# mokemokechicken/reversi-alpha-zero

Measured on NVIDIA H100. Metric: self_play_games_per_sec, higher is better.
Workload: dtype f16

## Files before the change

include/rz_engine.h:

```cpp
#ifndef RZ_ENGINE_H
#define RZ_ENGINE_H

#include <stddef.h>
#include <stdint.h>

#ifdef __cplusplus
extern "C" {
#endif

#define RZ_OK 0
#define RZ_EINVAL (-1)
#define RZ_ECUDA (-2)
#define RZ_ENOMEM (-3)
#define RZ_ESTATE (-4)
#define RZ_ECAPACITY (-5)
#define RZ_EIO (-6)

#define RZ_ABI_VERSION 2

int rz_abi_version(void);
const char* rz_last_error(void);
int rz_device_count(int* count);


int rz_find_correct_moves_dev(const uint64_t* own, const uint64_t* enemy, uint64_t* out, size_t n, void* stream);
int rz_find_correct_moves(const uint64_t* own, const uint64_t* enemy, uint64_t* out, size_t n);

int rz_calc_flip_dev(const uint8_t* pos, const uint64_t* own, const uint64_t* enemy, uint64_t* out, size_t n, void* stream);
int rz_calc_flip(const uint8_t* pos, const uint64_t* own, const uint64_t* enemy, uint64_t* out, size_t n);

int rz_step_dev(uint64_t* black, uint64_t* white, uint8_t* next_player, uint8_t* turn, uint8_t* done,
                uint8_t* winner, const int8_t* action, uint64_t* legal_out, size_t n, void* stream);
int rz_step(uint64_t* black, uint64_t* white, uint8_t* next_player, uint8_t* turn, uint8_t* done,
            uint8_t* winner, const int8_t* action, uint64_t* legal_out, size_t n);

int rz_dihedral_dev(const uint64_t* x, const uint8_t* t, uint64_t* out, size_t n, void* stream);

int rz_solve_dev(const uint64_t* own, const uint64_t* enemy, const uint8_t* exactly, int8_t* move, int8_t* score, size_t n,
                 void* stream);
int rz_solve(const uint64_t* own, const uint64_t* enemy, const uint8_t* exactly, int8_t* move, int8_t* score, size_t n);

typedef struct rz_deep_solve_stats {
    int32_t probes;
    int32_t slices;
    int32_t resplits;
    int32_t pad;
    int64_t leaves;
    int64_t node_steps;
    double seconds;
} rz_deep_solve_stats;
int rz_solve_deep(const uint64_t* own, const uint64_t* enemy, int8_t* move, int8_t* score, size_t n, double timeout_s,
                  rz_deep_solve_stats* stats);
int rz_solve_deep_tune(int slice_us, int leaf_target, int leaf_floor);

typedef struct rz_env_state {
    uint64_t black, white;
    uint8_t next_player, turn, done, winner;
} rz_env_state;
uint64_t rz_find_correct_moves_host(uint64_t own, uint64_t enemy);
uint64_t rz_calc_flip_host(int pos, uint64_t own, uint64_t enemy);
uint64_t rz_dihedral_host(uint64_t x, int t);
int rz_bitsliced_host(const uint8_t* pos, const uint64_t* own, const uint64_t* enemy, uint64_t* out, size_t n);
void rz_env_reset_host(rz_env_state* s);
void rz_env_update_host(rz_env_state* s, uint64_t black, uint64_t white, int next_player);
void rz_env_step_host(rz_env_state* s, int action );

typedef struct rz_net rz_net;

typedef struct rz_net_cfg {
    int32_t filters;
    int32_t res_blocks;
    int32_t value_fc;
    int32_t kernel_size;
} rz_net_cfg;

#define RZ_NET_IMPL_AUTO 0
#define RZ_NET_IMPL_GENERIC 1
#define RZ_NET_IMPL_TCGEN05 2
#define RZ_NET_IMPL_SPLIT 3

int rz_net_set_tower_cluster(int cluster);
int rz_net_create(const rz_net_cfg* cfg, int device, rz_net** out);
int rz_net_destroy(rz_net* net);
int rz_net_blob_size(const rz_net* net, size_t* n_floats);
int rz_net_load_weights(rz_net* net, const float* blob_host, size_t n_floats);
int rz_net_load_weights_dev(rz_net* net, const float* blob_dev, size_t n_floats, void* stream);

int rz_net_predict_dev(rz_net* net, const uint64_t* own, const uint64_t* enemy, float* policy, float* value,
                       size_t n, int impl, void* stream);
int rz_net_predict_counted_dev(rz_net* net, const uint64_t* own, const uint64_t* enemy, float* policy, float* value,
                               const uint32_t* count_dev, size_t max_n, int impl, void* stream);
int rz_net_debug_tower_dev(rz_net* net, const uint64_t* own, const uint64_t* enemy, float* policy, float* value,
                           float* tower, size_t n, void* stream);
int rz_net_debug_heads_dev(rz_net* net, const uint64_t* own, const uint64_t* enemy, float* policy, float* value,
                           float* tower, float* policy_logits, float* value_logit, size_t n, void* stream);
int rz_net_debug_heads_impl_dev(rz_net* net, const uint64_t* own, const uint64_t* enemy, float* policy, float* value,
                                float* tower, float* policy_logits, float* value_logit, size_t n, int impl, void* stream);
int rz_net_select_impl(const rz_net* net, size_t n, int* impl);
int rz_net_predict(rz_net* net, const uint8_t* planes, float* policy, float* value, size_t n, int impl);

typedef struct rz_engine rz_engine;

#define RZ_EVAL_NET 0
#define RZ_EVAL_FAKE 1

typedef struct rz_engine_cfg {
    int32_t games;
    int32_t simulation_num_per_move;
    int32_t parallel_search_num;
    int32_t virtual_loss;
    int32_t change_tau_turn;
    int32_t thinking_loop;
    int32_t required_visit_to_decide_action;
    int32_t start_rethinking_turn;
    int32_t allowed_resign_turn;
    int32_t use_resign_threshold;
    int32_t share_mtcs_info;
    int32_t eval_mode;
    int32_t net_impl;
    int32_t max_plies;
    int32_t warm_start;
    int32_t overlap_groups;
    int32_t max_sims_per_wave;
    int32_t use_solver_turn;
    int32_t use_solver_turn_in_simulation;
    int32_t reset_mtcs_info_per_game;
    int32_t max_searches_per_game;
    int32_t arena_simulation_num;
    int32_t eval_cache_mb;
    float c_puct;
    float noise_eps;
    float dirichlet_alpha;
    float resign_threshold;
    float disable_resignation_rate;
    uint64_t seed;
    uint64_t first_game_id;
    uint64_t game_id_stride;
    uint64_t max_games;
} rz_engine_cfg;

typedef struct rz_ply {
    uint64_t own, enemy;
    int32_t n_visit[64];
    int16_t action;
    uint8_t player;
    uint8_t loops;
    uint8_t recorded;
    uint8_t pad;
    uint16_t waves;
    float n;
    float q;
} rz_ply;

typedef struct rz_game {
    uint64_t game_id;
    uint64_t black, white;
    int32_t first_ply;
    int32_t n_plies;
    int32_t expansions;
    int32_t simulations;
    uint8_t winner;
    int8_t black_z;
    uint8_t resign_enabled;
    uint8_t resigned_mask;
    uint8_t turn;
    uint8_t black_net;
    uint8_t pad[2];
    int32_t table_nodes;
    int32_t pad2;
} rz_game;

typedef struct rz_stats {
    uint64_t games_started, games_finished;
    uint64_t expansions;
    uint64_t simulations;
    uint64_t waves;
    uint64_t plies;
    uint64_t nn_launches, mcts_launches;
    uint64_t max_nodes_used, max_edges_used;
    double nn_ms, mcts_ms;
    double run_ms;
    uint64_t tower_rows;
    uint64_t cache_lookups;
    uint64_t cache_hits;
    uint64_t cache_repeats;
} rz_stats;

int rz_engine_create(const rz_engine_cfg* cfg, rz_net* net , int device,
                     rz_engine** out);
int rz_engine_destroy(rz_engine* e);
int rz_engine_run(rz_engine* e, uint64_t finished_target, uint64_t max_waves);
int rz_engine_poll(rz_engine* e, rz_game* games, size_t game_cap, size_t* n_games, rz_ply* plies, size_t ply_cap,
                   size_t* n_plies);
int rz_engine_stats(rz_engine* e, rz_stats* out);
int rz_engine_cache_turn_stats(rz_engine* e, uint64_t* lookups, uint64_t* hits, int n);
int rz_engine_set_max_games(rz_engine* e, uint64_t max_games);
int rz_engine_set_warm_start_profile(rz_engine* e, const float* weight, int n);
int rz_engine_set_simulation_num(rz_engine* e, int32_t sims);
int rz_engine_set_second_net(rz_engine* e, rz_net* net_b, int enable);
int rz_engine_set_resign_threshold(rz_engine* e, int use_resign_threshold, float resign_threshold);
int rz_engine_search_root(rz_engine* e, uint64_t own, uint64_t enemy, int player, int slot, int keep_tree,
                          int32_t* n_visit, float* w_sum);

int rz_write_play_data(const char* path, const rz_game* games, size_t n_games, const rz_ply* plies,
                       int save_policy_of_tau_1, int change_tau_turn, size_t* n_records);

typedef struct rz_play_row {
    uint64_t own, enemy;
    int32_t n_visit[64];
    int32_t z;
    int32_t pad;
} rz_play_row;

int rz_write_play_rows(const char* path, const rz_game* games, size_t n_games, const rz_ply* plies,
                       int save_policy_of_tau_1, int change_tau_turn, size_t* n_rows);
int rz_read_play_rows(const char* path, rz_play_row* rows, size_t capacity, size_t* n_rows,
                      int* save_policy_of_tau_1, int* change_tau_turn);
int rz_ingest_dev(const rz_play_row* rows, size_t n_rows, int save_policy_of_tau_1, int change_tau_turn,
                  uint8_t* planes, float* policy, float* z, void* stream);
int rz_ingest(const rz_play_row* rows, size_t n_rows, int save_policy_of_tau_1, int change_tau_turn,
              uint8_t* planes, float* policy, float* z);

int rz_ingest_json_dev(const char* text, size_t n_bytes, size_t capacity, uint8_t* planes, float* policy, float* z,
                       size_t* n_records, size_t* error_offset, void* stream);
int rz_ingest_json_host(const char* text, size_t n_bytes, size_t capacity, uint8_t* planes, float* policy, float* z,
                        size_t* n_records, size_t* error_offset);
int rz_ingest_json(const char* path, size_t capacity, uint8_t* planes, float* policy, float* z, size_t* n_records,
                   size_t* error_offset);

typedef struct rz_trainer rz_trainer;

typedef struct rz_train_cfg {
    int32_t max_batch;
    float momentum;
    float l2_reg;
    float bn_momentum;
} rz_train_cfg;

int rz_trainer_create(const rz_net_cfg* net, const rz_train_cfg* cfg, int device, rz_trainer** out);
int rz_trainer_create_group(const rz_net_cfg* net, const rz_train_cfg* cfg, const int* devices, int n_devices, rz_trainer** out);
int rz_train_shard_plan_host(int filters, int res_blocks, int batch, int n_devices, int32_t* bounds);
int rz_trainer_destroy(rz_trainer* t);
int rz_trainer_blob_size(const rz_trainer* t, size_t* n_floats);
int rz_trainer_load_weights(rz_trainer* t, const float* blob_host, size_t n_floats);
int rz_trainer_load_weights_dev(rz_trainer* t, const float* blob_dev, size_t n_floats, void* stream);
int rz_trainer_weights_dev(rz_trainer* t, float* blob_dev, size_t n_floats, void* stream);
int rz_trainer_step_dev(rz_trainer* t, const uint8_t* planes, const float* policy, const float* z, size_t n_records,
                        const int32_t* index, size_t batch, float lr, float* loss_dev, void* stream);
int rz_trainer_last_grad_dev(rz_trainer* t, float* grad_dev, size_t n_floats, void* stream);
int rz_trainer_replica_state_dev(rz_trainer* t, int r, float* blob_dev, float* vel_dev, size_t n_floats, void* stream);

#define RZ_TRAIN_CONV0_FWD 0
#define RZ_TRAIN_CONV_FWD 1
#define RZ_TRAIN_CONV_DGRAD 2
#define RZ_TRAIN_CONV_WGRAD 3
#define RZ_TRAIN_CONV0_WGRAD 4
int rz_trainer_debug_conv_dev(rz_trainer* t, int op, const float* in, const float* kernel, const float* bias, const float* add,
                              size_t batch, float* out, void* stream);

#define RZ_TRAIN_T_X0 0
#define RZ_TRAIN_T_Y 1
#define RZ_TRAIN_T_A 2
#define RZ_TRAIN_T_STATS 3
#define RZ_TRAIN_T_STAT 4
#define RZ_TRAIN_T_HC 5
#define RZ_TRAIN_T_AH 6
#define RZ_TRAIN_T_DH 7
#define RZ_TRAIN_T_DYH 8
#define RZ_TRAIN_T_HP 9
#define RZ_TRAIN_T_HV 10
#define RZ_TRAIN_T_DL 11
#define RZ_TRAIN_T_H1 12
#define RZ_TRAIN_T_DH1 13
#define RZ_TRAIN_T_DV 14
#define RZ_TRAIN_T_LP 15
#define RZ_TRAIN_T_LV 16
#define RZ_TRAIN_T_LOSS_PV 17
#define RZ_TRAIN_T_G 18
#define RZ_TRAIN_T_DY 19
#define RZ_TRAIN_T_DZ 20
int rz_trainer_debug_tensor_dev(rz_trainer* t, int which, int layer, float* out, size_t n_floats, void* stream);
int rz_trainer_debug_keep_backward(rz_trainer* t, int on);

#ifdef __cplusplus
}
#endif
#endif
```

reversi-alpha-zero_b200/csrc/rz_net.cu:

```cuda
#include <math.h>
#include <stdlib.h>
#include <string.h>
#include <new>
#include "rz_bitboard.cuh"
#include "rz_net.cuh"
#include "rz_tc_common.cuh"

namespace rz {

constexpr float kBnEps = 1e-3f;

__global__ void fold_bn_kernel(const float* __restrict__ blob, size_t group_off, size_t kernel_floats, int cout,
                               float* __restrict__ scale, float* __restrict__ shift) {
    int c = blockIdx.x * blockDim.x + threadIdx.x;
    if (c >= cout) return;
    const float* p = blob + group_off + kernel_floats;
    float bias = p[c], gamma = p[cout + c], beta = p[2 * cout + c], mean = p[3 * cout + c], var = p[4 * cout + c];
    float s = gamma / sqrtf(var + kBnEps);
    scale[c] = s;
    shift[c] = beta + (bias - mean) * s;
}

constexpr int kGThreads = 256;

template <int PIX>
__device__ __forceinline__ void conv3x3_layer(const float* __restrict__ in, float* __restrict__ out, const float* __restrict__ w,
                                              const float* __restrict__ scale, const float* __restrict__ shift, int cin, int F,
                                              bool add_residual, int oc, int pg, bool active) {
    float acc[PIX];
#pragma unroll
    for (int i = 0; i < PIX; ++i) acc[i] = 0.f;
    if (active) {
        for (int ci = 0; ci < cin; ++ci) {
            const float* inc = in + ci * 100;
#pragma unroll
            for (int tap = 0; tap < 9; ++tap) {
                const float wv = __ldg(w + ((size_t)tap * cin + ci) * F + oc);
                const int dy = tap / 3, dx = tap % 3;
#pragma unroll
                for (int i = 0; i < PIX; ++i) {
                    const int p = pg * PIX + i;
                    acc[i] = fmaf(inc[((p >> 3) + dy) * 10 + (p & 7) + dx], wv, acc[i]);
                }
            }
        }
        const float s = scale[oc], b = shift[oc];
#pragma unroll
        for (int i = 0; i < PIX; ++i) {
            const int p = pg * PIX + i;
            const int o = oc * 100 + ((p >> 3) + 1) * 10 + (p & 7) + 1;
            float y = fmaf(acc[i], s, b);
            if (add_residual) y += out[o];
            out[o] = fmaxf(y, 0.f);
        }
    }
}

template <int PIX>
__global__ void __launch_bounds__(kGThreads) net_generic_kernel(const float* __restrict__ blob, const float* __restrict__ ss,
                                                                rz_net net, const u64* __restrict__ own, const u64* __restrict__ enemy,
                                                                float* __restrict__ policy, float* __restrict__ value, size_t n,
                                                                const uint32_t* __restrict__ n_dev) {
    extern __shared__ float smem[];
    if (n_dev) n = *n_dev;
    const int F = net.cfg.filters, R = net.cfg.res_blocks, V = net.cfg.value_fc;
    float* bufA = smem;
    float* bufB = smem + F * 100;
    float* hp = bufB + F * 100;
    float* hv = hp + 128;
    float* fc = hv + 64;
    const int t = threadIdx.x;
    constexpr int NPG = 64 / PIX;
    const int oc = t % F, pg = t / F;
    const bool active = (t < F * NPG) && (pg < NPG);

    for (size_t pos = blockIdx.x; pos < n; pos += gridDim.x) {
        for (int i = t; i < 2 * F * 100; i += kGThreads) smem[i] = 0.f;
        __syncthreads();
        const u64 o = own[pos], e = enemy[pos];
        if (t < 128) {
            const int c = t >> 6, p = t & 63;
            bufB[c * 100 + ((p >> 3) + 1) * 10 + (p & 7) + 1] = (float)(((c ? e : o) >> p) & 1ULL);
        }
        __syncthreads();
        conv3x3_layer<PIX>(bufB, bufA, blob + net.off_conv0, ss, ss + F, 2, F, false, oc, pg, active);
        __syncthreads();
        for (int r = 0; r < R; ++r) {
            const float* w1 = blob + net.off_res0 + (size_t)(2 * r) * net.res_stride_conv;
            const float* w2 = w1 + net.res_stride_conv;
            const float* ss1 = ss + (size_t)(1 + 2 * r) * 2 * F;
            const float* ss2 = ss1 + 2 * F;
            conv3x3_layer<PIX>(bufA, bufB, w1, ss1, ss1 + F, F, F, false, oc, pg, active);
            __syncthreads();
            conv3x3_layer<PIX>(bufB, bufA, w2, ss2, ss2 + F, F, F, true, oc, pg, active);
            __syncthreads();
        }
        const float* ssh = ss + (size_t)(1 + 2 * R) * 2 * F;
        if (t < 192) {
            const int c = t >> 6, p = t & 63;
            const float* w = c < 2 ? blob + net.off_policy_conv + c : blob + net.off_value_conv;
            const int wstride = c < 2 ? 2 : 1;
            float acc = 0.f;
            const int o2 = ((p >> 3) + 1) * 10 + (p & 7) + 1;
            for (int ci = 0; ci < F; ++ci) acc = fmaf(bufA[ci * 100 + o2], __ldg(w + (size_t)ci * wstride), acc);
            if (c < 2) hp[c * 64 + p] = fmaxf(fmaf(acc, ssh[c], ssh[2 + c]), 0.f);
            else       hv[p] = fmaxf(fmaf(acc, ssh[4], ssh[5]), 0.f);
        }
        __syncthreads();
        if (t < 64) {
            const float* k = blob + net.off_policy_fc_k;
            float acc = __ldg(blob + net.off_policy_fc_b + t);
            for (int i = 0; i < 128; ++i) acc = fmaf(hp[i], __ldg(k + i * 64 + t), acc);
            fc[t] = acc;
        }
        __syncthreads();
        if (t < 64) {
            float m = -INFINITY;
            for (int i = 0; i < 64; ++i) m = fmaxf(m, fc[i]);
            float sum = 0.f;
            for (int i = 0; i < 64; ++i) sum += expf(fc[i] - m);
            policy[pos * 64 + t] = expf(fc[t] - m) / sum;
        }
        __syncthreads();
        for (int j = t; j < V; j += kGThreads) {
            const float* k = blob + net.off_value_fc1_k;
            float acc = __ldg(blob + net.off_value_fc1_b + j);
            for (int i = 0; i < 64; ++i) acc = fmaf(hv[i], __ldg(k + (size_t)i * V + j), acc);
            fc[j] = fmaxf(acc, 0.f);
        }
        __syncthreads();
        if (t == 0) {
            float acc = __ldg(blob + net.off_value_fc2_b);
            for (int j = 0; j < V; ++j) acc = fmaf(fc[j], __ldg(blob + net.off_value_fc2_k + j), acc);
            value[pos] = tanhf(acc);
        }
        __syncthreads();
    }
}

int net_forward_generic(rz_net* net, const uint64_t* own, const uint64_t* enemy, float* policy, float* value, size_t n,
                        cudaStream_t stream, const uint32_t* n_dev) {
    const int F = net->cfg.filters, V = net->cfg.value_fc;
    RZ_REQUIRE(F >= 2 && F <= 256, "generic kernel supports 2 <= filters <= 256 (got %d)", F);
    const size_t smem = ((size_t)2 * F * 100 + 128 + 64 + (V > 64 ? V : 64)) * sizeof(float);
    int npg = kGThreads / F;
    int pix = 64;
    while (pix > 4 && 64 / (pix / 2) <= npg) pix /= 2;
    size_t blocks = n < (size_t)num_sms() * 2 ? n : (size_t)num_sms() * 2;
    if (smem > 110 * 1024) blocks = n < (size_t)num_sms() ? n : (size_t)num_sms();
#define RZ_LAUNCH_G(P)                                                                                             \
    do {                                                                                                           \
        RZ_CUDA_TRY(cudaFuncSetAttribute(net_generic_kernel<P>, cudaFuncAttributeMaxDynamicSharedMemorySize, (int)smem)); \
        net_generic_kernel<P><<<(unsigned)blocks, kGThreads, smem, stream>>>(net->blob, net->scale_shift, *net, own, enemy, policy, value, n, n_dev); \
    } while (0)
    switch (pix) {
        case 64: RZ_LAUNCH_G(64); break;
        case 32: RZ_LAUNCH_G(32); break;
        case 16: RZ_LAUNCH_G(16); break;
        case 8: RZ_LAUNCH_G(8); break;
        default: RZ_LAUNCH_G(4); break;
    }
#undef RZ_LAUNCH_G
    RZ_LAUNCH_CHECK();
    return RZ_OK;
}

constexpr size_t kSplitMaxBatch = 0;

int select_impl(const rz_net* net, size_t n, int impl) {
    if (impl != RZ_NET_IMPL_AUTO) return impl;
    if (!tc_width(net->cfg.filters) || net->cfg.value_fc > (int)tc::kTcMaxV) return RZ_NET_IMPL_GENERIC;
    if (net->cfg.filters != 256) return RZ_NET_IMPL_TCGEN05;
    return n <= kSplitMaxBatch ? RZ_NET_IMPL_SPLIT : RZ_NET_IMPL_TCGEN05;
}

int net_forward(rz_net* net, const uint64_t* own, const uint64_t* enemy, float* policy, float* value, size_t n, int impl,
                cudaStream_t stream) {
    if (!net->loaded) { set_error("rz_net: weights not loaded"); return RZ_ESTATE; }
    if (n == 0) return RZ_OK;
    impl = select_impl(net, n, impl);
    if (impl == RZ_NET_IMPL_TCGEN05 || impl == RZ_NET_IMPL_SPLIT) {
        if (impl == RZ_NET_IMPL_SPLIT) {
            RZ_REQUIRE(net->cfg.filters == 256, "the split tower requires filters == 256 (got %d)", net->cfg.filters);
            return net_forward_split(net, own, enemy, policy, value, n, stream, nullptr);
        }
        RZ_REQUIRE(tc_width(net->cfg.filters), "the tensor-core tower requires filters 64, 128 or 256 (got %d)", net->cfg.filters);
        return net_forward_tc(net, own, enemy, policy, value, n, stream, nullptr);
    }
    RZ_REQUIRE(impl == RZ_NET_IMPL_GENERIC, "unknown net impl %d", impl);
    return net_forward_generic(net, own, enemy, policy, value, n, stream);
}

int net_forward_counted(rz_net* net, const uint64_t* own, const uint64_t* enemy, float* policy, float* value,
                        const uint32_t* count_dev, size_t max_n, int impl, cudaStream_t stream) {
    if (!net->loaded) { set_error("rz_net: weights not loaded"); return RZ_ESTATE; }
    impl = select_impl(net, max_n, impl);
    if (impl == RZ_NET_IMPL_TCGEN05) return net_forward_tc(net, own, enemy, policy, value, max_n, stream, nullptr, count_dev);
    if (impl == RZ_NET_IMPL_SPLIT) return net_forward_split(net, own, enemy, policy, value, max_n, stream, nullptr, count_dev);
    return net_forward_generic(net, own, enemy, policy, value, max_n, stream, count_dev);
}

static int finish_load(rz_net* net, cudaStream_t stream) {
    const rz_net_cfg& c = net->cfg;
    const int F = c.filters, L = n_conv_layers(c);
    float* ss = net->scale_shift;
    for (int l = 0; l < L; ++l) {
        const size_t off = l == 0 ? net->off_conv0 : net->off_res0 + (size_t)(l - 1) * net->res_stride_conv;
        const size_t kf = l == 0 ? (size_t)9 * 2 * F : (size_t)9 * F * F;
        fold_bn_kernel<<<(F + 127) / 128, 128, 0, stream>>>(net->blob, off, kf, F, ss + (size_t)l * 2 * F, ss + (size_t)l * 2 * F + F);
    }
    float* ssh = ss + (size_t)L * 2 * F;
    fold_bn_kernel<<<1, 32, 0, stream>>>(net->blob, net->off_policy_conv, (size_t)F * 2, 2, ssh, ssh + 2);
    fold_bn_kernel<<<1, 32, 0, stream>>>(net->blob, net->off_value_conv, (size_t)F, 1, ssh + 4, ssh + 5);
    RZ_LAUNCH_CHECK();
    if (F == 256) RZ_TRY(net_pack_tc(net, stream));
    else if (tc_width(F)) RZ_TRY(net_pack_tc_narrow(net, stream));
    RZ_CUDA_TRY(cudaStreamSynchronize(stream));
    net->loaded = true;
    net->weights_version++;
    return RZ_OK;
}

}

using namespace rz;

extern "C" {

int rz_net_create(const rz_net_cfg* cfg, int device, rz_net** out) {
    RZ_REQUIRE(cfg && out, "rz_net_create: null pointer");
    RZ_REQUIRE(cfg->kernel_size == 3, "only cnn_filter_size == 3 is supported (got %d)", cfg->kernel_size);
    RZ_REQUIRE(cfg->filters >= 2 && cfg->filters <= 256 && cfg->res_blocks >= 0 && cfg->res_blocks <= 64 && cfg->value_fc >= 1 &&
                   cfg->value_fc <= 4096,
               "unsupported model configuration (filters=%d res_blocks=%d value_fc=%d)", cfg->filters, cfg->res_blocks, cfg->value_fc);
    RZ_CUDA_TRY(cudaSetDevice(device));
    rz_net* net = new (std::nothrow) rz_net();
    if (!net) { set_error("out of host memory"); return RZ_ENOMEM; }
    memset(net, 0, sizeof(*net));
    net->cfg = *cfg;
    net->device = device;
    const size_t F = cfg->filters, V = cfg->value_fc, R = cfg->res_blocks;
    size_t off = 0;
    net->off_conv0 = off; off += 9 * 2 * F + 5 * F;
    net->off_res0 = off; net->res_stride_conv = 9 * F * F + 5 * F; off += 2 * R * net->res_stride_conv;
    net->off_policy_conv = off; off += F * 2 + 5 * 2;
    net->off_policy_fc_k = off; off += 128 * 64;
    net->off_policy_fc_b = off; off += 64;
    net->off_value_conv = off; off += F + 5;
    net->off_value_fc1_k = off; off += 64 * V;
    net->off_value_fc1_b = off; off += V;
    net->off_value_fc2_k = off; off += V;
    net->off_value_fc2_b = off; off += 1;
    net->blob_floats = off;
    cudaError_t e = cudaMalloc(&net->blob, off * sizeof(float));
    if (e == cudaSuccess) e = cudaMalloc(&net->scale_shift, ss_floats(*cfg) * sizeof(float));
    if (e == cudaSuccess && tc_width((int)F)) {
        e = cudaMalloc(&net->tc_w0, (size_t)4 * F * 8 * sizeof(__half));
        if (e == cudaSuccess && R > 0) e = cudaMalloc(&net->tc_w, (size_t)2 * R * 9 * F * F * sizeof(__half));
        if (e == cudaSuccess) e = cudaMalloc(&net->res, (size_t)num_sms() * kTowerResFloatsPerCta * sizeof(float));
        if (e == cudaSuccess) e = cudaEventCreateWithFlags(&net->res_done, cudaEventDisableTiming);
    }
    if (e != cudaSuccess) {
        set_error("rz_net_create: cudaMalloc failed: %s", cudaGetErrorString(e));
        cudaGetLastError();
        rz_net_destroy(net);
        return RZ_ENOMEM;
    }
    *out = net;
    return RZ_OK;
}

int rz_net_destroy(rz_net* net) {
    if (!net) return RZ_OK;
    cudaSetDevice(net->device);
    cudaFree(net->blob); cudaFree(net->scale_shift); cudaFree(net->tc_w0); cudaFree(net->tc_w); cudaFree(net->scratch);
    cudaFree(net->res); cudaFree(net->feat);
    if (net->res_done) cudaEventDestroy(net->res_done);
    delete net;
    return RZ_OK;
}

int rz_net_blob_size(const rz_net* net, size_t* n_floats) {
    RZ_REQUIRE(net && n_floats, "rz_net_blob_size: null pointer");
    *n_floats = net->blob_floats;
    return RZ_OK;
}

int rz_net_load_weights(rz_net* net, const float* blob_host, size_t n_floats) {
    RZ_REQUIRE(net && blob_host, "rz_net_load_weights: null pointer");
    RZ_REQUIRE(n_floats == net->blob_floats, "weight blob has %zu floats, this configuration needs %zu", n_floats, net->blob_floats);
    RZ_CUDA_TRY(cudaSetDevice(net->device));
    RZ_CUDA_TRY(cudaMemcpy(net->blob, blob_host, n_floats * sizeof(float), cudaMemcpyHostToDevice));
    return finish_load(net, 0);
}

int rz_net_load_weights_dev(rz_net* net, const float* blob_dev, size_t n_floats, void* stream) {
    RZ_REQUIRE(net && blob_dev, "rz_net_load_weights_dev: null pointer");
    RZ_REQUIRE(n_floats == net->blob_floats, "weight blob has %zu floats, this configuration needs %zu", n_floats, net->blob_floats);
    RZ_CUDA_TRY(cudaSetDevice(net->device));
    RZ_CUDA_TRY(cudaMemcpyAsync(net->blob, blob_dev, n_floats * sizeof(float), cudaMemcpyDeviceToDevice, (cudaStream_t)stream));
    return finish_load(net, (cudaStream_t)stream);
}

int rz_net_set_tower_cluster(int cluster) { return set_tower_cluster(cluster); }

int rz_net_predict_dev(rz_net* net, const uint64_t* own, const uint64_t* enemy, float* policy, float* value, size_t n, int impl,
                       void* stream) {
    RZ_REQUIRE(net && (n == 0 || (own && enemy && policy && value)), "rz_net_predict_dev: null pointer");
    return net_forward(net, own, enemy, policy, value, n, impl, (cudaStream_t)stream);
}

int rz_net_predict_counted_dev(rz_net* net, const uint64_t* own, const uint64_t* enemy, float* policy, float* value,
                               const uint32_t* count_dev, size_t max_n, int impl, void* stream) {
    RZ_REQUIRE(net && count_dev && (max_n == 0 || (own && enemy && policy && value)), "rz_net_predict_counted_dev: null pointer");
    if (max_n == 0) return RZ_OK;
    return net_forward_counted(net, own, enemy, policy, value, count_dev, max_n, impl, (cudaStream_t)stream);
}

int rz_net_debug_tower_dev(rz_net* net, const uint64_t* own, const uint64_t* enemy, float* policy, float* value, float* tower, size_t n,
                           void* stream) {
    RZ_REQUIRE(net && own && enemy && policy && value && tower, "rz_net_debug_tower_dev: null pointer");
    if (!net->loaded) { set_error("rz_net: weights not loaded"); return RZ_ESTATE; }
    return net_forward_tc(net, own, enemy, policy, value, n, (cudaStream_t)stream, tower);
}

int rz_net_debug_heads_dev(rz_net* net, const uint64_t* own, const uint64_t* enemy, float* policy, float* value, float* tower,
                           float* policy_logits, float* value_logit, size_t n, void* stream) {
    RZ_REQUIRE(net && own && enemy && policy && value && policy_logits && value_logit, "rz_net_debug_heads_dev: null pointer");
    if (!net->loaded) { set_error("rz_net: weights not loaded"); return RZ_ESTATE; }
    return net_forward_tc(net, own, enemy, policy, value, n, (cudaStream_t)stream, tower, nullptr, policy_logits, value_logit);
}

int rz_net_debug_heads_impl_dev(rz_net* net, const uint64_t* own, const uint64_t* enemy, float* policy, float* value, float* tower,
                                float* policy_logits, float* value_logit, size_t n, int impl, void* stream) {
    RZ_REQUIRE(net && own && enemy && policy && value && policy_logits && value_logit, "rz_net_debug_heads_impl_dev: null pointer");
    if (!net->loaded) { set_error("rz_net: weights not loaded"); return RZ_ESTATE; }
    RZ_REQUIRE(tc_width(net->cfg.filters), "the tensor-core tower requires filters 64, 128 or 256 (got %d)", net->cfg.filters);
    if (n == 0) return RZ_OK;
    impl = select_impl(net, n, impl);
    if (impl == RZ_NET_IMPL_SPLIT)
        return net_forward_split(net, own, enemy, policy, value, n, (cudaStream_t)stream, tower, nullptr, policy_logits, value_logit);
    RZ_REQUIRE(impl == RZ_NET_IMPL_TCGEN05, "rz_net_debug_heads_impl_dev: impl must be AUTO, TCGEN05 or SPLIT (got %d)", impl);
    return net_forward_tc(net, own, enemy, policy, value, n, (cudaStream_t)stream, tower, nullptr, policy_logits, value_logit);
}

int rz_net_select_impl(const rz_net* net, size_t n, int* impl) {
    RZ_REQUIRE(net && impl, "rz_net_select_impl: null pointer");
    *impl = select_impl(net, n, RZ_NET_IMPL_AUTO);
    return RZ_OK;
}

int rz_net_predict(rz_net* net, const uint8_t* planes, float* policy, float* value, size_t n, int impl) {
    RZ_REQUIRE(net && (n == 0 || (planes && policy && value)), "rz_net_predict: null pointer");
    if (n == 0) return RZ_OK;
    RZ_CUDA_TRY(cudaSetDevice(net->device));
    const size_t need = n * (16 + 65 * 4) + 256;
    if (need > net->scratch_bytes) {
        cudaFree(net->scratch); net->scratch = nullptr; net->scratch_bytes = 0;
        RZ_CUDA_TRY(cudaMalloc(&net->scratch, need));
        net->scratch_bytes = need;
    }
    uint64_t* hb = (uint64_t*)malloc(n * 16);
    if (!hb) { set_error("out of host memory"); return RZ_ENOMEM; }
    for (size_t i = 0; i < n; ++i) {
        uint64_t o = 0, e = 0;
        const uint8_t* p = planes + i * 128;
        for (int b = 0; b < 64; ++b) { o |= (uint64_t)(p[b] != 0) << b; e |= (uint64_t)(p[64 + b] != 0) << b; }
        hb[i] = o; hb[n + i] = e;
    }
    uint64_t* d_own = (uint64_t*)net->scratch;
    uint64_t* d_en = d_own + n;
    float* d_pol = (float*)(d_en + n);
    float* d_val = d_pol + n * 64;
    cudaError_t ce = cudaMemcpyAsync(d_own, hb, n * 16, cudaMemcpyHostToDevice, 0);
    int rc = RZ_OK;
    if (ce == cudaSuccess) rc = net_forward(net, d_own, d_en, d_pol, d_val, n, impl, 0);
    if (ce == cudaSuccess && rc == RZ_OK) ce = cudaMemcpyAsync(policy, d_pol, n * 64 * sizeof(float), cudaMemcpyDeviceToHost, 0);
    if (ce == cudaSuccess && rc == RZ_OK) ce = cudaMemcpyAsync(value, d_val, n * sizeof(float), cudaMemcpyDeviceToHost, 0);
    if (ce == cudaSuccess && rc == RZ_OK) ce = cudaStreamSynchronize(0);
    free(hb);
    if (rc != RZ_OK) return rc;
    if (ce != cudaSuccess) { set_error("rz_net_predict: %s", cudaGetErrorString(ce)); return RZ_ECUDA; }
    return RZ_OK;
}

}
```

reversi-alpha-zero_b200/csrc/rz_net.cuh:

```cuda
#pragma once
#include <cuda_fp16.h>
#include <mutex>
#include "rz_common.cuh"

struct rz_net {
    rz_net_cfg cfg;
    int device;
    bool loaded;
    uint64_t weights_version;
    size_t blob_floats;
    float* blob;
    float* scale_shift;
    size_t off_conv0, off_res0, res_stride_conv;
    size_t off_policy_conv, off_policy_fc_k, off_policy_fc_b;
    size_t off_value_conv, off_value_fc1_k, off_value_fc1_b, off_value_fc2_k, off_value_fc2_b;
    __half* tc_w0;
    __half* tc_w;
    float* res;
    cudaEvent_t res_done;
    float* feat;
    size_t feat_rows;
    void* scratch;
    size_t scratch_bytes;
};

namespace rz {

constexpr size_t kTowerResFloatsPerCta = 256 * 128;
constexpr int kHeadFeatures = 192;

inline int n_conv_layers(const rz_net_cfg& c) { return 1 + 2 * c.res_blocks; }
inline size_t ss_floats(const rz_net_cfg& c) { return (size_t)n_conv_layers(c) * 2 * c.filters + 4 + 2; }

int net_forward_generic(rz_net* net, const uint64_t* own, const uint64_t* enemy, float* policy, float* value, size_t n,
                        cudaStream_t stream, const uint32_t* n_dev = nullptr);
int net_forward_counted(rz_net* net, const uint64_t* own, const uint64_t* enemy, float* policy, float* value,
                        const uint32_t* count_dev, size_t max_n, int impl, cudaStream_t stream);
int net_forward_tc(rz_net* net, const uint64_t* own, const uint64_t* enemy, float* policy, float* value, size_t n,
                   cudaStream_t stream, float* dbg_tower ,
                   const uint32_t* n_dev = nullptr ,
                   float* dbg_logits = nullptr , float* dbg_vlogit = nullptr );
int net_forward_split(rz_net* net, const uint64_t* own, const uint64_t* enemy, float* policy, float* value, size_t n,
                      cudaStream_t stream, float* dbg_tower, const uint32_t* n_dev = nullptr, float* dbg_logits = nullptr,
                      float* dbg_vlogit = nullptr);
int select_impl(const rz_net* net, size_t n, int impl);
int net_pack_tc(rz_net* net, cudaStream_t stream);
std::mutex& tower_mutex();
int head_features(rz_net* net, size_t n);
int net_forward_tc_narrow(rz_net* net, const uint64_t* own, const uint64_t* enemy, float* policy, float* value, size_t n,
                          cudaStream_t stream, float* dbg_tower, const uint32_t* n_dev, float* dbg_logits, float* dbg_vlogit);
int net_pack_tc_narrow(rz_net* net, cudaStream_t stream);
inline bool tc_width(int filters) { return filters == 64 || filters == 128 || filters == 256; }
int set_tower_cluster(int cluster);
int tower_cluster();
int net_forward(rz_net* net, const uint64_t* own, const uint64_t* enemy, float* policy, float* value, size_t n, int impl,
                cudaStream_t stream);

}
```

reversi-alpha-zero_b200/csrc/rz_net_tc.cu:

```cuda
#include <stdlib.h>
#include <mutex>
#include <type_traits>
#include "rz_bitboard.cuh"
#include "rz_net.cuh"
#include "rz_tc_common.cuh"

namespace rz {
namespace tc {

constexpr int kThreads = 384;
constexpr uint32_t kProducerRegs = 40, kMathRegs = 232;
constexpr int kMathThreads = 256;
constexpr uint32_t kActCg = 2896, kActSlot = 144;
constexpr uint32_t kActBytes = 32 * kActCg;
constexpr uint32_t kStageBytes = 32768, kStages = 3;
constexpr int kResAhead = 4;
constexpr uint32_t kA0Bytes = 8192, kW0Bytes = 16384;
constexpr uint32_t kOffAct = 0;
constexpr uint32_t kOffW = kOffAct + kActBytes;
constexpr uint32_t kOffA0 = kOffW + kStages * kStageBytes;
constexpr uint32_t kOffW0 = kOffA0 + kA0Bytes;
constexpr uint32_t kOffSS = kOffW0 + kW0Bytes;
constexpr uint32_t kOffHw = kOffSS + 2 * 2048;
constexpr uint32_t kOffBar = kOffHw + 768 * 4;
constexpr uint32_t kNumBars = 2 * kStages + 1;
constexpr uint32_t kSmemBytes = kOffBar + kNumBars * 8;
constexpr uint32_t kSmemAlloc = kSmemBytes + 128;
static_assert(kSmemAlloc <= 232448, "shared memory budget exceeded");
static_assert(kTowerResFloatsPerCta == (size_t)kMathThreads * 128, "residual scratch per CTA");

#ifdef RZ_TOWER_STAMPS
enum : int {
    kStTiles,
    kStTile,
    kStKLoop,
    kStFull,
    kStMma,
    kStEpiBar,
    kStEpi0,
    kStEpi1,
    kStEpi2,
    kStEpiLast,
    kStFeat,
    kStEmpty,
    kStCount
};
constexpr int kStMaxCtas = 1024;
__device__ unsigned long long g_tower_stamps[kStMaxCtas][kStCount];
__device__ __forceinline__ void stamp_add(int phase, uint32_t cycles) { atomicAdd(&g_tower_stamps[blockIdx.x][phase], (unsigned long long)cycles); }
#define RZ_STAMP(...) __VA_ARGS__
#else
#define RZ_STAMP(...)
#endif

template <int CL>
__global__ void __launch_bounds__(kThreads, 1) net_tower_kernel(const Params pp) {
    Params p = pp;
    if (p.n_dev) p.n = *p.n_dev;
    extern __shared__ uint8_t smem_raw[];
    const uint32_t base = (smem_u32(smem_raw) + 127u) & ~127u;
    uint8_t* sm = smem_raw + (base - smem_u32(smem_raw));
    const int warp = threadIdx.x >> 5, lane = threadIdx.x & 31;
    const uint32_t bar0 = base + kOffBar;
    auto bar_full = [&](uint32_t s) { return bar0 + s * 8; };
    auto bar_empty = [&](uint32_t s) { return bar0 + (kStages + s) * 8; };
    const uint32_t bar_w0 = bar0 + 2 * kStages * 8;
    const uint32_t ntiles = (p.n + 1) >> 1;
    const int L = p.n_layers;
    const uint32_t crank = CL > 1 ? cluster_ctarank() : 0u;
    const uint32_t cbase = blockIdx.x - crank;
    const uint32_t iters = cbase < ntiles ? (ntiles - cbase + gridDim.x - 1) / gridDim.x : 0u;

    for (uint32_t i = threadIdx.x * 16; i < kActBytes; i += kThreads * 16) *reinterpret_cast<uint4*>(sm + kOffAct + i) = make_uint4(0, 0, 0, 0);
    fence_proxy_async();
    for (uint32_t i = threadIdx.x; i < 768; i += kThreads)
        reinterpret_cast<float*>(sm + kOffHw)[i] = __ldg(i < 512 ? p.blob + p.off_policy_conv + i : p.blob + p.off_value_conv + (i - 512));
    if (threadIdx.x == 0) {
        for (uint32_t s = 0; s < kStages; ++s) { mbar_init(bar_full(s), 1); mbar_init(bar_empty(s), 8 * CL); }
        mbar_init(bar_w0, 1);
        asm volatile("fence.mbarrier_init.release.cluster;" ::: "memory");
    }
    __syncthreads();
    if (CL > 1) cluster_sync_all();

    if (warp >= 8) {
        asm volatile("setmaxnreg.dec.sync.aligned.u32 %0;" ::"n"(kProducerRegs));
        if (warp == 8 && lane == 0) {
            if (iters > 0) {
                mbar_expect_tx(bar_w0, kW0Bytes);
                bulk_g2s(base + kOffW0, p.w0, kW0Bytes, bar_w0);
            }
            uint32_t stage = 0, phase = 0;
            for (uint32_t it = 0; it < iters; ++it) {
                for (int l = 1; l < L; ++l) {
                    const uint8_t* src = reinterpret_cast<const uint8_t*>(p.w) + (size_t)(l - 1) * 36 * kStageBytes;
                    RZ_STAMP(uint32_t st_empty = 0;)
                    for (int s = 0; s < 36; ++s) {
                        RZ_STAMP(const uint32_t c0 = (uint32_t)clock();)
                        mbar_wait(bar_empty(stage), phase ^ 1);
                        RZ_STAMP(st_empty += (uint32_t)clock() - c0;)
                        mbar_expect_tx(bar_full(stage), kStageBytes);
                        if (CL == 1) {
                            bulk_g2s(base + kOffW + stage * kStageBytes, src + (size_t)s * kStageBytes, kStageBytes, bar_full(stage));
                        } else {
                            constexpr uint32_t kSlice = kStageBytes / CL;
                            bulk_g2s_mc(base + kOffW + stage * kStageBytes + crank * kSlice, src + (size_t)s * kStageBytes + crank * kSlice,
                                        kSlice, bar_full(stage), (uint16_t)((1u << CL) - 1u));
                        }
                        if (++stage == kStages) { stage = 0; phase ^= 1; }
                    }
                    RZ_STAMP(stamp_add(kStEmpty, st_empty);)
                }
            }
        }
    } else {
        asm volatile("setmaxnreg.inc.sync.aligned.u32 %0;" ::"n"(kMathRegs));
        const int et = threadIdx.x;
        const int wg = warp >> 2;
        const int r0 = wg * 64 + (warp & 3) * 16 + (lane >> 2);
        const int g0 = r0 >> 3, x = r0 & 7, y = g0 >> 1;
        const int cq = 2 * (lane & 3);
        const uint32_t act_row0 = base + kOffAct + (g0 + 2) * kActSlot + (x + 1) * 16 + cq * 2;
        const uint32_t act_row1 = act_row0 + kActSlot;
        const uint32_t a_wg = base + kOffAct + wg * 8 * kActSlot;
        float* ss_s = reinterpret_cast<float*>(sm + kOffSS);
        float4* res = reinterpret_cast<float4*>(p.res + (size_t)blockIdx.x * kTowerResFloatsPerCta) + et;
        const float* hw = reinterpret_cast<const float*>(sm + kOffHw);
        uint32_t stage = 0, phase = 0, ss_buf = 0;
        float d[128];
        ss_s[et] = __ldg(p.ss + et);
        ss_s[256 + et] = __ldg(p.ss + 256 + et);

        for (uint32_t it = 0; it < iters; ++it) {
            const uint32_t tile = blockIdx.x + it * gridDim.x;
            const uint32_t pos0 = tile * 2;
            RZ_STAMP(const uint32_t st_tile0 = (uint32_t)clock();)
            {
                const int m = et & 127, g = m >> 3, brd = g & 1;
                const bool valid = pos0 + brd < p.n;
                build_layer0_operand(sm + kOffA0, valid ? p.own[pos0 + brd] : 0, valid ? p.enemy[pos0 + brd] : 0, 2 * (et >> 7), g, m & 7,
                                     g >> 1);
                fence_proxy_async();
            }
            float hs[6];
            for (int l = 0; l < L; ++l) {
                const float* sc = ss_s + ss_buf * 512;
                const bool is_conv2 = l > 0 && (l & 1) == 0;
                float4 rb[kResAhead];
                RZ_STAMP(uint32_t st_c = (uint32_t)clock(), st_bar = 0, st_full = 0, st_mma = 0;)
                epi_bar();
                RZ_STAMP(st_bar += (uint32_t)clock() - st_c;)
                {
                    const size_t nl = l + 1 < L ? (size_t)l + 1 : 0;
                    const uint32_t dst = smem_u32(ss_s + (ss_buf ^ 1) * 512 + et);
                    cp_async_4(dst, p.ss + nl * 512 + et);
                    cp_async_4(dst + 1024, p.ss + nl * 512 + 256 + et);
                }
                RZ_STAMP(const uint32_t st_k0 = (uint32_t)clock();)
                acc_fence(d);
                if (l == 0) {
                    RZ_STAMP(st_c = (uint32_t)clock();)
                    mbar_wait(bar_w0, 0);
                    RZ_STAMP(st_full += (uint32_t)clock() - st_c;)
                    wgmma_fence();
#pragma unroll
                    for (uint32_t j = 0; j < 2; ++j)
                        wgmma_m64n256k16(d, smem_desc(base + kOffA0 + j * 2 * 2048 + wg * 1024, 2048, 128),
                                         smem_desc(base + kOffW0 + j * 2 * 4096, 4096, 128), j);
                    wgmma_commit();
                    RZ_STAMP(st_c = (uint32_t)clock();)
                    wgmma_wait<0>();
                    RZ_STAMP(st_mma += (uint32_t)clock() - st_c;)
                } else {
                    int prev = -1;
                    for (uint32_t tap = 0; tap < 9; ++tap) {
                        const uint32_t a_tap = a_wg + (2 * (tap / 3)) * kActSlot + (tap % 3) * 16;
                        for (uint32_t kb = 0; kb < 4; ++kb) {
                            RZ_STAMP(st_c = (uint32_t)clock();)
                            mbar_wait(bar_full(stage), phase);
                            RZ_STAMP(st_full += (uint32_t)clock() - st_c;)
                            const uint32_t b_st = base + kOffW + stage * kStageBytes;
                            wgmma_fence();
#pragma unroll
                            for (uint32_t j = 0; j < 4; ++j)
                                wgmma_m64n256k16(d, smem_desc(a_tap + (kb * 8 + 2 * j) * kActCg, kActCg, kActSlot),
                                                 smem_desc(b_st + 2 * j * 4096, 4096, 128), (tap | kb | j) != 0);
                            wgmma_commit();
                            RZ_STAMP(st_c = (uint32_t)clock();)
                            wgmma_wait<1>();
                            RZ_STAMP(st_mma += (uint32_t)clock() - st_c;)
                            if (prev >= 0 && lane == 0) {
                                mbar_arrive(bar_empty(prev));
                                if (CL > 1) mbar_arrive_cta(bar_empty(prev), crank ^ 1u);
                            }
                            prev = (int)stage;
                            if (++stage == kStages) { stage = 0; phase ^= 1; }
                        }
                    }
                    if (is_conv2) {
#pragma unroll
                        for (int i = 0; i < kResAhead; ++i) rb[i] = res[i * 256];
                    }
                    RZ_STAMP(st_c = (uint32_t)clock();)
                    wgmma_wait<0>();
                    RZ_STAMP(st_mma += (uint32_t)clock() - st_c;)
                    if (lane == 0) {
                        mbar_arrive(bar_empty(prev));
                        if (CL > 1) mbar_arrive_cta(bar_empty(prev), crank ^ 1u);
                    }
                }
                RZ_STAMP(const uint32_t st_k1 = (uint32_t)clock();)
                acc_fence(d);
                cp_async_wait_all();
                ss_buf ^= 1;
                const bool keep_res = l == 0 || is_conv2;
                const bool last = l == L - 1;
                RZ_STAMP(st_c = (uint32_t)clock();)
                if (!last) epi_bar();
                RZ_STAMP(const uint32_t st_e0 = (uint32_t)clock(); st_bar += st_e0 - st_c;)
                float* dbg0 = nullptr;
                float* dbg1 = nullptr;
                if (last && p.dbg_tower) {
                    if (pos0 < p.n) dbg0 = p.dbg_tower + ((size_t)pos0 * 64 + y * 8 + x) * 256;
                    if (pos0 + 1 < p.n) dbg1 = p.dbg_tower + ((size_t)(pos0 + 1) * 64 + y * 8 + x) * 256;
                }
                constexpr int kEpiRelu = 0, kEpiKeep = 1, kEpiLast = 2;
                auto epilogue = [&](auto conv2, auto kind) {
                    constexpr bool kConv2 = decltype(conv2)::value;
                    constexpr bool kKeep = decltype(kind)::value == kEpiKeep, kLast = decltype(kind)::value == kEpiLast;
                    if (kLast) {
#pragma unroll
                        for (int k = 0; k < 6; ++k) hs[k] = 0.f;
                    }
#pragma unroll
                for (int i = 0; i < 32; ++i) {
                    const int c = 8 * i + cq;
                    const float2 s = *reinterpret_cast<const float2*>(sc + c);
                    const float2 b = *reinterpret_cast<const float2*>(sc + 256 + c);
                    float v0 = fmaf(d[4 * i + 0], s.x, b.x), v1 = fmaf(d[4 * i + 1], s.y, b.y);
                    float v2 = fmaf(d[4 * i + 2], s.x, b.x), v3 = fmaf(d[4 * i + 3], s.y, b.y);
                    if (kConv2) {
                        const float4 r = rb[i % kResAhead];
                        if (i + kResAhead < 32) rb[i % kResAhead] = res[(i + kResAhead) * 256];
                        v0 += r.x; v1 += r.y; v2 += r.z; v3 += r.w;
                    }
                    if (kKeep || kLast) {
                        v0 = fmaxf(v0, 0.f); v1 = fmaxf(v1, 0.f); v2 = fmaxf(v2, 0.f); v3 = fmaxf(v3, 0.f);
                    }
                    if (!kLast) {
                        if (kKeep) res[i * 256] = make_float4(v0, v1, v2, v3);
                        const uint32_t h0 = pack_h2<!kKeep>(v0, v1);
                        const uint32_t h1 = pack_h2<!kKeep>(v2, v3);
                        const uint32_t off = (c >> 3) * kActCg;
                        asm volatile("st.shared.b32 [%0], %1;" ::"r"(act_row0 + off), "r"(h0) : "memory");
                        asm volatile("st.shared.b32 [%0], %1;" ::"r"(act_row1 + off), "r"(h1) : "memory");
                    } else {
                        const float4 w = *reinterpret_cast<const float4*>(hw + 2 * c);
                        const float2 wv = *reinterpret_cast<const float2*>(hw + 512 + c);
                        hs[0] = fmaf(v1, w.z, fmaf(v0, w.x, hs[0]));
                        hs[1] = fmaf(v1, w.w, fmaf(v0, w.y, hs[1]));
                        hs[2] = fmaf(v1, wv.y, fmaf(v0, wv.x, hs[2]));
                        hs[3] = fmaf(v3, w.z, fmaf(v2, w.x, hs[3]));
                        hs[4] = fmaf(v3, w.w, fmaf(v2, w.y, hs[4]));
                        hs[5] = fmaf(v3, wv.y, fmaf(v2, wv.x, hs[5]));
                        if (dbg0) *reinterpret_cast<float2*>(dbg0 + c) = make_float2(v0, v1);
                        if (dbg1) *reinterpret_cast<float2*>(dbg1 + c) = make_float2(v2, v3);
                    }
                }
                };
                using Conv2 = std::true_type;
                using NoConv2 = std::false_type;
                if (last) {
                    if (is_conv2) epilogue(Conv2(), std::integral_constant<int, kEpiLast>());
                    else epilogue(NoConv2(), std::integral_constant<int, kEpiLast>());
                } else if (is_conv2) {
                    epilogue(Conv2(), std::integral_constant<int, kEpiKeep>());
                } else if (keep_res) {
                    epilogue(NoConv2(), std::integral_constant<int, kEpiKeep>());
                } else {
                    epilogue(NoConv2(), std::integral_constant<int, kEpiRelu>());
                }
                if (!last) fence_proxy_async();
                RZ_STAMP(if (et == 0) {
                    stamp_add(kStKLoop, st_k1 - st_k0); stamp_add(kStFull, st_full); stamp_add(kStMma, st_mma); stamp_add(kStEpiBar, st_bar);
                    stamp_add(l == 0 ? kStEpi0 : last ? kStEpiLast : is_conv2 ? kStEpi2 : kStEpi1, (uint32_t)clock() - st_e0);
                })
            }
            RZ_STAMP(const uint32_t st_h0 = (uint32_t)clock();)
#pragma unroll
            for (int k = 0; k < 6; ++k) {
                hs[k] += __shfl_xor_sync(0xffffffffu, hs[k], 1);
                hs[k] += __shfl_xor_sync(0xffffffffu, hs[k], 2);
            }
            {
                const int q = lane & 3;
                if (q < 2 && pos0 + q < p.n) {
                    const float h0 = q ? hs[3] : hs[0], h1 = q ? hs[4] : hs[1], h2 = q ? hs[5] : hs[2];
                    store_head_features(p.feat + (size_t)(pos0 + q) * kHeadFeatures, p.ss + (size_t)L * 512, y * 8 + x, h0 + 0.f,
                                        h1 + 0.f, h2 + 0.f);
                }
            }
            RZ_STAMP(if (et == 0) {
                const uint32_t st_h1 = (uint32_t)clock();
                stamp_add(kStFeat, st_h1 - st_h0); stamp_add(kStTile, st_h1 - st_tile0); stamp_add(kStTiles, 1);
            })
        }
    }

    __syncthreads();
    if (CL > 1) cluster_sync_all();
}

__global__ void pack_w0_kernel(const float* __restrict__ k0, __half* __restrict__ out) {
    const int i = blockIdx.x * blockDim.x + threadIdx.x;
    if (i >= 4 * 256 * 8) return;
    const int j = i & 7, n = (i >> 3) & 255, kc = i >> 11, k = kc * 8 + j;
    out[i] = __float2half_rn(k < 18 ? k0[(size_t)k * 256 + n] : 0.f);
}
__global__ void pack_w_kernel(const float* __restrict__ blob, size_t off_res0, size_t stride, int n_layers, __half* __restrict__ out) {
    const size_t total = (size_t)n_layers * 36 * 8 * 256 * 8;
    for (size_t i = (size_t)blockIdx.x * blockDim.x + threadIdx.x; i < total; i += (size_t)gridDim.x * blockDim.x) {
        const int j = i & 7, n = (i >> 3) & 255, kc = (i >> 11) & 7;
        const size_t ls = i >> 14;
        const int s = (int)(ls % 36), l = (int)(ls / 36);
        const int tap = s >> 2, kb = s & 3, ci = kb * 64 + kc * 8 + j;
        out[i] = __float2half_rn(blob[off_res0 + (size_t)l * stride + ((size_t)tap * 256 + ci) * 256 + n]);
    }
}

}

int net_pack_tc(rz_net* net, cudaStream_t stream) {
    tc::pack_w0_kernel<<<(4 * 256 * 8 + 255) / 256, 256, 0, stream>>>(net->blob + net->off_conv0, net->tc_w0);
    if (net->cfg.res_blocks > 0)
        tc::pack_w_kernel<<<num_sms() * 8, 256, 0, stream>>>(net->blob, net->off_res0, net->res_stride_conv, 2 * net->cfg.res_blocks, net->tc_w);
    RZ_LAUNCH_CHECK();
    return RZ_OK;
}

static int g_cluster = 0;

int set_tower_cluster(int cluster) {
    RZ_REQUIRE(cluster == 1 || cluster == 2, "rz_net_set_tower_cluster: cluster must be 1 or 2");
    g_cluster = cluster;
    return RZ_OK;
}

int tower_cluster() {
    if (g_cluster == 0) {
        const char* cs = getenv("RZ_TOWER_CLUSTER");
        g_cluster = (cs && atoi(cs) == 1) ? 1 : 2;
    }
    return g_cluster;
}

int net_forward_tc(rz_net* net, const uint64_t* own, const uint64_t* enemy, float* policy, float* value, size_t n, cudaStream_t stream,
                   float* dbg_tower, const uint32_t* n_dev, float* dbg_logits, float* dbg_vlogit) {
    if (net->cfg.filters == 64 || net->cfg.filters == 128)
        return net_forward_tc_narrow(net, own, enemy, policy, value, n, stream, dbg_tower, n_dev, dbg_logits, dbg_vlogit);
    RZ_REQUIRE(net->cfg.filters == 256, "wgmma tower requires 64, 128 or 256 filters (got %d)", net->cfg.filters);
    RZ_REQUIRE(net->cfg.value_fc <= (int)tc::kTcMaxV, "wgmma tower supports value_fc_size <= %u", tc::kTcMaxV);
    RZ_REQUIRE(n < (1ull << 31), "batch too large");
    static int max_pairs = -1;
    if (max_pairs < 0) {
        RZ_CUDA_TRY(cudaFuncSetAttribute(tc::net_tower_kernel<1>, cudaFuncAttributeMaxDynamicSharedMemorySize, (int)tc::kSmemAlloc));
        RZ_CUDA_TRY(cudaFuncSetAttribute(tc::net_tower_kernel<2>, cudaFuncAttributeMaxDynamicSharedMemorySize, (int)tc::kSmemAlloc));
        cudaLaunchConfig_t cfg = {};
        cfg.gridDim = dim3((unsigned)num_sms() & ~1u); cfg.blockDim = dim3(tc::kThreads); cfg.dynamicSmemBytes = tc::kSmemAlloc;
        cudaLaunchAttribute attr[1];
        attr[0].id = cudaLaunchAttributeClusterDimension;
        attr[0].val.clusterDim.x = 2; attr[0].val.clusterDim.y = 1; attr[0].val.clusterDim.z = 1;
        cfg.attrs = attr; cfg.numAttrs = 1;
        RZ_CUDA_TRY(cudaOccupancyMaxActiveClusters(&max_pairs, tc::net_tower_kernel<2>, &cfg));
    }
    const int cluster = tower_cluster() == 2 && max_pairs >= 1 ? 2 : 1;
    tc::Params p;
    p.w0 = net->tc_w0; p.w = net->tc_w; p.ss = net->scale_shift; p.blob = net->blob;
    p.off_policy_conv = net->off_policy_conv; p.off_policy_fc_k = net->off_policy_fc_k; p.off_policy_fc_b = net->off_policy_fc_b;
    p.off_value_conv = net->off_value_conv; p.off_value_fc1_k = net->off_value_fc1_k; p.off_value_fc1_b = net->off_value_fc1_b;
    p.off_value_fc2_k = net->off_value_fc2_k; p.off_value_fc2_b = net->off_value_fc2_b;
    p.own = own; p.enemy = enemy; p.policy = policy; p.value = value; p.dbg_tower = dbg_tower;
    p.dbg_logits = dbg_logits; p.dbg_vlogit = dbg_vlogit;
    p.n = (uint32_t)n; p.n_dev = n_dev; p.n_layers = 1 + 2 * net->cfg.res_blocks; p.V = net->cfg.value_fc;
    p.res = net->res;
    std::lock_guard<std::mutex> lock(tower_mutex());
    RZ_TRY(head_features(net, n));
    p.feat = net->feat;
    RZ_CUDA_TRY(cudaStreamWaitEvent(stream, net->res_done, 0));
    const uint32_t ntiles = (uint32_t)((n + 1) / 2);
    uint32_t grid = ntiles < (uint32_t)num_sms() ? ntiles : (uint32_t)num_sms();
    if (cluster == 1) {
        tc::net_tower_kernel<1><<<grid, tc::kThreads, tc::kSmemAlloc, stream>>>(p);
    } else {
        grid = (grid + 1) & ~1u;
        if (grid > 2u * (uint32_t)max_pairs) grid = 2u * (uint32_t)max_pairs;
        cudaLaunchConfig_t cfg = {};
        cfg.gridDim = dim3(grid); cfg.blockDim = dim3(tc::kThreads); cfg.dynamicSmemBytes = tc::kSmemAlloc; cfg.stream = stream;
        cudaLaunchAttribute attr[1];
        attr[0].id = cudaLaunchAttributeClusterDimension;
        attr[0].val.clusterDim.x = 2; attr[0].val.clusterDim.y = 1; attr[0].val.clusterDim.z = 1;
        cfg.attrs = attr; cfg.numAttrs = 1;
        RZ_CUDA_TRY(cudaLaunchKernelEx(&cfg, tc::net_tower_kernel<2>, p));
    }
    RZ_LAUNCH_CHECK();
    RZ_TRY(net_heads(p, stream));
    RZ_CUDA_TRY(cudaEventRecord(net->res_done, stream));
    return RZ_OK;
}

}

#ifdef RZ_TOWER_STAMPS
extern "C" int rz_tower_stamps(unsigned long long* out, int n_ctas, int reset) {
    using namespace rz::tc;
    if (n_ctas < 0 || n_ctas > kStMaxCtas) return (int)cudaErrorInvalidValue;
    const size_t bytes = (size_t)n_ctas * kStCount * sizeof(unsigned long long);
    cudaError_t e = cudaDeviceSynchronize();
    if (e == cudaSuccess && out) e = cudaMemcpyFromSymbol(out, g_tower_stamps, bytes);
    if (e == cudaSuccess && reset) {
        void* dev = nullptr;
        e = cudaGetSymbolAddress(&dev, g_tower_stamps);
        if (e == cudaSuccess) e = cudaMemset(dev, 0, sizeof(g_tower_stamps));
        if (e == cudaSuccess) e = cudaDeviceSynchronize();
    }
    return (int)e;
}
extern "C" int rz_tower_stamp_count() { return rz::tc::kStCount; }
#endif
```

reversi-alpha-zero_b200/csrc/rz_tc_common.cuh:

```cuda
#pragma once
#include <cuda_fp16.h>
#include "rz_bitboard.cuh"
#include "rz_net.cuh"

namespace rz {
namespace tc {

__device__ __forceinline__ uint32_t smem_u32(const void* p) { return (uint32_t)__cvta_generic_to_shared(p); }

__device__ __forceinline__ void mbar_init(uint32_t bar, uint32_t count) {
    asm volatile("mbarrier.init.shared::cta.b64 [%0], %1;" ::"r"(bar), "r"(count) : "memory");
}
__device__ __forceinline__ void mbar_expect_tx(uint32_t bar, uint32_t bytes) {
    asm volatile("mbarrier.arrive.expect_tx.shared::cta.b64 _, [%0], %1;" ::"r"(bar), "r"(bytes) : "memory");
}
__device__ __forceinline__ void mbar_arrive(uint32_t bar) {
    asm volatile("mbarrier.arrive.shared::cta.b64 _, [%0];" ::"r"(bar) : "memory");
}
__device__ __forceinline__ void mbar_arrive_cta(uint32_t bar, uint32_t rank) {
    uint32_t remote;
    asm volatile("mapa.shared::cluster.u32 %0, %1, %2;" : "=r"(remote) : "r"(bar), "r"(rank));
    asm volatile("mbarrier.arrive.shared::cluster.b64 _, [%0];" ::"r"(remote) : "memory");
}
__device__ __forceinline__ void mbar_wait(uint32_t bar, uint32_t parity) {
    uint32_t ok = 0;
    long long t0 = 0;
    for (uint32_t spin = 0; !ok; ++spin) {
        asm volatile(
            "{\n\t.reg .pred p;\n\t"
            "mbarrier.try_wait.parity.shared::cta.b64 p, [%1], %2;\n\t"
            "selp.u32 %0, 1, 0, p;\n\t}"
            : "=r"(ok)
            : "r"(bar), "r"(parity)
            : "memory");
        if (!ok && (spin & 1023) == 1023) {
            const long long now = clock64();
            if (t0 == 0) t0 = now;
            else if (now - t0 > 8000000000LL) __trap();
        }
    }
}
__device__ __forceinline__ void bulk_g2s(uint32_t dst, const void* src, uint32_t bytes, uint32_t bar) {
    asm volatile("cp.async.bulk.shared::cluster.global.mbarrier::complete_tx::bytes [%0], [%1], %2, [%3];" ::"r"(dst), "l"(src),
                 "r"(bytes), "r"(bar)
                 : "memory");
}
__device__ __forceinline__ void bulk_g2s_mc(uint32_t dst, const void* src, uint32_t bytes, uint32_t bar, uint16_t mask) {
    asm volatile(
        "cp.async.bulk.shared::cluster.global.mbarrier::complete_tx::bytes.multicast::cluster [%0], [%1], %2, [%3], %4;" ::"r"(dst),
        "l"(src), "r"(bytes), "r"(bar), "h"(mask)
        : "memory");
}
__device__ __forceinline__ void cluster_sync_all() {
    asm volatile("barrier.cluster.arrive.release.aligned;\n\tbarrier.cluster.wait.acquire.aligned;" ::: "memory");
}
__device__ __forceinline__ uint32_t cluster_ctarank() {
    uint32_t r;
    asm volatile("mov.u32 %0, %%cluster_ctarank;" : "=r"(r));
    return r;
}
__device__ __forceinline__ void cp_async_4(uint32_t dst, const void* src) {
    asm volatile("cp.async.ca.shared.global [%0], [%1], 4;" ::"r"(dst), "l"(src) : "memory");
}
__device__ __forceinline__ void cp_async_wait_all() { asm volatile("cp.async.wait_all;" ::: "memory"); }
__device__ __forceinline__ void fence_proxy_async() { asm volatile("fence.proxy.async.shared::cta;" ::: "memory"); }
__device__ __forceinline__ void epi_bar() { asm volatile("bar.sync 1, 256;" ::: "memory"); }

__device__ __forceinline__ uint64_t smem_desc(uint32_t addr, uint32_t lbo, uint32_t sbo) {
    return (uint64_t)((addr >> 4) & 0x3FFF) | ((uint64_t)((lbo >> 4) & 0x3FFF) << 16) | ((uint64_t)((sbo >> 4) & 0x3FFF) << 32);
}
__device__ __forceinline__ void wgmma_fence() { asm volatile("wgmma.fence.sync.aligned;" ::: "memory"); }
__device__ __forceinline__ void wgmma_commit() { asm volatile("wgmma.commit_group.sync.aligned;" ::: "memory"); }
template <int N>
__device__ __forceinline__ void wgmma_wait() { asm volatile("wgmma.wait_group.sync.aligned %0;" ::"n"(N) : "memory"); }
__device__ __forceinline__ void acc_fence(float (&d)[128]) {
#pragma unroll
    for (int i = 0; i < 128; ++i) asm volatile("" : "+f"(d[i])::"memory");
}

#define RZ_D4(i) "+f"(d[i]), "+f"(d[i + 1]), "+f"(d[i + 2]), "+f"(d[i + 3])
#define RZ_D16(i) RZ_D4(i), RZ_D4(i + 4), RZ_D4(i + 8), RZ_D4(i + 12)
__device__ __forceinline__ void wgmma_m64n256k16(float (&d)[128], uint64_t adesc, uint64_t bdesc, uint32_t accumulate) {
    asm volatile(
        "{\n\t.reg .pred p;\n\t"
        "setp.ne.b32 p, %130, 0;\n\t"
        "wgmma.mma_async.sync.aligned.m64n256k16.f32.f16.f16 {"
        "%0, %1, %2, %3, %4, %5, %6, %7, %8, %9, %10, %11, %12, %13, %14, %15, "
        "%16, %17, %18, %19, %20, %21, %22, %23, %24, %25, %26, %27, %28, %29, %30, %31, "
        "%32, %33, %34, %35, %36, %37, %38, %39, %40, %41, %42, %43, %44, %45, %46, %47, "
        "%48, %49, %50, %51, %52, %53, %54, %55, %56, %57, %58, %59, %60, %61, %62, %63, "
        "%64, %65, %66, %67, %68, %69, %70, %71, %72, %73, %74, %75, %76, %77, %78, %79, "
        "%80, %81, %82, %83, %84, %85, %86, %87, %88, %89, %90, %91, %92, %93, %94, %95, "
        "%96, %97, %98, %99, %100, %101, %102, %103, %104, %105, %106, %107, %108, %109, %110, %111, "
        "%112, %113, %114, %115, %116, %117, %118, %119, %120, %121, %122, %123, %124, %125, %126, %127"
        "}, %128, %129, p, 1, 1, 0, 0;\n\t}"
        : RZ_D16(0), RZ_D16(16), RZ_D16(32), RZ_D16(48), RZ_D16(64), RZ_D16(80), RZ_D16(96), RZ_D16(112)
        : "l"(adesc), "l"(bdesc), "r"(accumulate)
        : "memory");
}
template <int O>
__device__ __forceinline__ void wgmma_m64n128k16(float (&d)[128], uint64_t adesc, uint64_t bdesc, uint32_t accumulate) {
    asm volatile(
        "{\n\t.reg .pred p;\n\t"
        "setp.ne.b32 p, %66, 0;\n\t"
        "wgmma.mma_async.sync.aligned.m64n128k16.f32.f16.f16 {"
        "%0, %1, %2, %3, %4, %5, %6, %7, %8, %9, %10, %11, %12, %13, %14, %15, "
        "%16, %17, %18, %19, %20, %21, %22, %23, %24, %25, %26, %27, %28, %29, %30, %31, "
        "%32, %33, %34, %35, %36, %37, %38, %39, %40, %41, %42, %43, %44, %45, %46, %47, "
        "%48, %49, %50, %51, %52, %53, %54, %55, %56, %57, %58, %59, %60, %61, %62, %63"
        "}, %64, %65, p, 1, 1, 0, 0;\n\t}"
        : RZ_D16(O), RZ_D16(O + 16), RZ_D16(O + 32), RZ_D16(O + 48)
        : "l"(adesc), "l"(bdesc), "r"(accumulate)
        : "memory");
}
template <int O>
__device__ __forceinline__ void wgmma_m64n64k16(float (&d)[128], uint64_t adesc, uint64_t bdesc, uint32_t accumulate) {
    asm volatile(
        "{\n\t.reg .pred p;\n\t"
        "setp.ne.b32 p, %34, 0;\n\t"
        "wgmma.mma_async.sync.aligned.m64n64k16.f32.f16.f16 {"
        "%0, %1, %2, %3, %4, %5, %6, %7, %8, %9, %10, %11, %12, %13, %14, %15, "
        "%16, %17, %18, %19, %20, %21, %22, %23, %24, %25, %26, %27, %28, %29, %30, %31"
        "}, %32, %33, p, 1, 1, 0, 0;\n\t}"
        : RZ_D16(O), RZ_D16(O + 16)
        : "l"(adesc), "l"(bdesc), "r"(accumulate)
        : "memory");
}
#undef RZ_D16
#undef RZ_D4

template <bool RELU>
__device__ __forceinline__ uint32_t pack_h2(float a, float b) {
    uint32_t d;
    if (RELU) asm("cvt.rn.relu.satfinite.f16x2.f32 %0, %1, %2;" : "=r"(d) : "f"(b), "f"(a));
    else      asm("cvt.rn.satfinite.f16x2.f32 %0, %1, %2;" : "=r"(d) : "f"(b), "f"(a));
    return d;
}

struct Params {
    const __half* w0;
    const __half* w;
    const float* ss;
    const float* blob;
    size_t off_policy_conv, off_policy_fc_k, off_policy_fc_b, off_value_conv, off_value_fc1_k, off_value_fc1_b, off_value_fc2_k,
        off_value_fc2_b;
    const u64* own;
    const u64* enemy;
    float* policy;
    float* value;
    float* res;
    float* feat;
    float* dbg_tower;
    float* dbg_logits;
    float* dbg_vlogit;
    uint32_t n;
    const uint32_t* n_dev;
    int n_layers;
    int V;
};

constexpr uint32_t kTcMaxV = 512;

__device__ __forceinline__ void build_layer0_operand(uint8_t* a0, u64 o, u64 e, int kc0, int g, int x, int y) {
#pragma unroll
    for (int kk = 0; kk < 2; ++kk) {
        const int kc = kc0 + kk;
        uint32_t w[4];
#pragma unroll
        for (int jp = 0; jp < 4; ++jp) {
            uint32_t packed = 0;
#pragma unroll
            for (int half = 0; half < 2; ++half) {
                const int k = kc * 8 + jp * 2 + half;
                uint32_t bit = 0;
                if (k < 18) {
                    const int tap = k >> 1, yy = y + tap / 3 - 1, xx = x + tap % 3 - 1;
                    if (yy >= 0 && yy < 8 && xx >= 0 && xx < 8) bit = (uint32_t)((((k & 1) ? e : o) >> (yy * 8 + xx)) & 1ULL);
                }
                packed |= (bit ? 0x3C00u : 0u) << (16 * half);
            }
            w[jp] = packed;
        }
        *reinterpret_cast<uint4*>(a0 + kc * 2048 + g * 128 + x * 16) = make_uint4(w[0], w[1], w[2], w[3]);
    }
}

__device__ __forceinline__ void store_head_features(float* f, const float* ssh, int pix, float a0, float a1, float av) {
    f[pix] = fmaxf(fmaf(a0, ssh[0], ssh[2]), 0.f);
    f[64 + pix] = fmaxf(fmaf(a1, ssh[1], ssh[3]), 0.f);
    f[128 + pix] = fmaxf(fmaf(av, ssh[4], ssh[5]), 0.f);
}

}

int net_heads(const tc::Params& p, cudaStream_t stream);

}
```

reversi-alpha-zero_b200/reversi_zero_b200/_cabi.py:

```python
import ctypes as C
import os

_HERE = os.path.dirname(os.path.abspath(__file__))
LIB_PATH = os.path.join(os.path.dirname(_HERE), "csrc", "librz_engine.so")

u64p, u8p, i8p, f32p, i32p = (C.POINTER(C.c_uint64), C.POINTER(C.c_uint8), C.POINTER(C.c_int8),
                              C.POINTER(C.c_float), C.POINTER(C.c_int32))
vp, sz = C.c_void_p, C.c_size_t


class RzError(RuntimeError):
    pass


class EnvState(C.Structure):
    _fields_ = [("black", C.c_uint64), ("white", C.c_uint64), ("next_player", C.c_uint8), ("turn", C.c_uint8),
                ("done", C.c_uint8), ("winner", C.c_uint8)]


class NetCfg(C.Structure):
    _fields_ = [("filters", C.c_int32), ("res_blocks", C.c_int32), ("value_fc", C.c_int32), ("kernel_size", C.c_int32)]


class TrainCfg(C.Structure):
    _fields_ = [("max_batch", C.c_int32), ("momentum", C.c_float), ("l2_reg", C.c_float), ("bn_momentum", C.c_float)]


class EngineCfg(C.Structure):
    _fields_ = [(n, C.c_int32) for n in (
        "games", "simulation_num_per_move", "parallel_search_num", "virtual_loss", "change_tau_turn", "thinking_loop",
        "required_visit_to_decide_action", "start_rethinking_turn", "allowed_resign_turn", "use_resign_threshold",
        "share_mtcs_info", "eval_mode", "net_impl", "max_plies", "warm_start", "overlap_groups", "max_sims_per_wave", "use_solver_turn", "use_solver_turn_in_simulation",
        "reset_mtcs_info_per_game", "max_searches_per_game", "arena_simulation_num", "eval_cache_mb")] + [(n, C.c_float) for n in (
            "c_puct", "noise_eps", "dirichlet_alpha", "resign_threshold", "disable_resignation_rate")] + [
        (n, C.c_uint64) for n in ("seed", "first_game_id", "game_id_stride", "max_games")]


class Ply(C.Structure):
    _fields_ = [("own", C.c_uint64), ("enemy", C.c_uint64), ("n_visit", C.c_int32 * 64), ("action", C.c_int16),
                ("player", C.c_uint8), ("loops", C.c_uint8), ("recorded", C.c_uint8), ("pad", C.c_uint8), ("waves", C.c_uint16),
                ("n", C.c_float), ("q", C.c_float)]


class Game(C.Structure):
    _fields_ = [("game_id", C.c_uint64), ("black", C.c_uint64), ("white", C.c_uint64), ("first_ply", C.c_int32),
                ("n_plies", C.c_int32), ("expansions", C.c_int32), ("simulations", C.c_int32), ("winner", C.c_uint8),
                ("black_z", C.c_int8), ("resign_enabled", C.c_uint8), ("resigned_mask", C.c_uint8), ("turn", C.c_uint8),
                ("black_net", C.c_uint8), ("pad", C.c_uint8 * 2), ("table_nodes", C.c_int32), ("pad2", C.c_int32)]


class PlayRow(C.Structure):
    _fields_ = [("own", C.c_uint64), ("enemy", C.c_uint64), ("n_visit", C.c_int32 * 64), ("z", C.c_int32), ("pad", C.c_int32)]


class DeepSolveStats(C.Structure):
    _fields_ = [("probes", C.c_int32), ("slices", C.c_int32), ("resplits", C.c_int32), ("pad", C.c_int32),
                ("leaves", C.c_int64), ("node_steps", C.c_int64), ("seconds", C.c_double)]


class Stats(C.Structure):
    _fields_ = [(n, C.c_uint64) for n in ("games_started", "games_finished", "expansions", "simulations", "waves",
                                          "plies", "nn_launches", "mcts_launches", "max_nodes_used", "max_edges_used")] + [
        ("nn_ms", C.c_double), ("mcts_ms", C.c_double), ("run_ms", C.c_double)] + [
        (n, C.c_uint64) for n in ("tower_rows", "cache_lookups", "cache_hits", "cache_repeats")]


SIGNATURES = {
    "rz_abi_version": (C.c_int, []),
    "rz_last_error": (C.c_char_p, []),
    "rz_device_count": (C.c_int, [C.POINTER(C.c_int)]),
    "rz_bitsliced_host": (C.c_int, [u8p, u64p, u64p, u64p, sz]),
    "rz_find_correct_moves_dev": (C.c_int, [vp, vp, vp, sz, vp]),
    "rz_find_correct_moves": (C.c_int, [u64p, u64p, u64p, sz]),
    "rz_calc_flip_dev": (C.c_int, [vp, vp, vp, vp, sz, vp]),
    "rz_calc_flip": (C.c_int, [u8p, u64p, u64p, u64p, sz]),
    "rz_step_dev": (C.c_int, [vp, vp, vp, vp, vp, vp, vp, vp, sz, vp]),
    "rz_step": (C.c_int, [u64p, u64p, u8p, u8p, u8p, u8p, i8p, u64p, sz]),
    "rz_dihedral_dev": (C.c_int, [vp, vp, vp, sz, vp]),
    "rz_solve_dev": (C.c_int, [vp, vp, vp, vp, vp, sz, vp]),
    "rz_solve": (C.c_int, [u64p, u64p, u8p, i8p, i8p, sz]),
    "rz_solve_deep": (C.c_int, [u64p, u64p, i8p, i8p, sz, C.c_double, C.POINTER(DeepSolveStats)]),
    "rz_solve_deep_tune": (C.c_int, [C.c_int, C.c_int, C.c_int]),
    "rz_find_correct_moves_host": (C.c_uint64, [C.c_uint64, C.c_uint64]),
    "rz_calc_flip_host": (C.c_uint64, [C.c_int, C.c_uint64, C.c_uint64]),
    "rz_dihedral_host": (C.c_uint64, [C.c_uint64, C.c_int]),
    "rz_env_reset_host": (None, [C.POINTER(EnvState)]),
    "rz_env_update_host": (None, [C.POINTER(EnvState), C.c_uint64, C.c_uint64, C.c_int]),
    "rz_env_step_host": (None, [C.POINTER(EnvState), C.c_int]),
    "rz_net_create": (C.c_int, [C.POINTER(NetCfg), C.c_int, C.POINTER(vp)]),
    "rz_net_destroy": (C.c_int, [vp]),
    "rz_net_blob_size": (C.c_int, [vp, C.POINTER(sz)]),
    "rz_net_load_weights": (C.c_int, [vp, f32p, sz]),
    "rz_net_load_weights_dev": (C.c_int, [vp, vp, sz, vp]),
    "rz_net_predict_dev": (C.c_int, [vp, vp, vp, vp, vp, sz, C.c_int, vp]),
    "rz_net_predict_counted_dev": (C.c_int, [vp, vp, vp, vp, vp, vp, sz, C.c_int, vp]),
    "rz_net_set_tower_cluster": (C.c_int, [C.c_int]),
    "rz_net_debug_tower_dev": (C.c_int, [vp, vp, vp, vp, vp, vp, sz, vp]),
    "rz_net_debug_heads_dev": (C.c_int, [vp, vp, vp, vp, vp, vp, vp, vp, sz, vp]),
    "rz_net_debug_heads_impl_dev": (C.c_int, [vp, vp, vp, vp, vp, vp, vp, vp, sz, C.c_int, vp]),
    "rz_net_select_impl": (C.c_int, [vp, sz, C.POINTER(C.c_int)]),
    "rz_net_predict": (C.c_int, [vp, u8p, f32p, f32p, sz, C.c_int]),
    "rz_engine_create": (C.c_int, [C.POINTER(EngineCfg), vp, C.c_int, C.POINTER(vp)]),
    "rz_engine_destroy": (C.c_int, [vp]),
    "rz_engine_run": (C.c_int, [vp, C.c_uint64, C.c_uint64]),
    "rz_engine_poll": (C.c_int, [vp, C.POINTER(Game), sz, C.POINTER(sz), C.POINTER(Ply), sz, C.POINTER(sz)]),
    "rz_engine_stats": (C.c_int, [vp, C.POINTER(Stats)]),
    "rz_engine_cache_turn_stats": (C.c_int, [vp, u64p, u64p, C.c_int]),
    "rz_engine_set_simulation_num": (C.c_int, [vp, C.c_int32]),
    "rz_engine_set_warm_start_profile": (C.c_int, [vp, f32p, C.c_int]),
    "rz_engine_set_max_games": (C.c_int, [vp, C.c_uint64]),
    "rz_engine_set_second_net": (C.c_int, [vp, vp, C.c_int]),
    "rz_engine_set_resign_threshold": (C.c_int, [vp, C.c_int, C.c_float]),
    "rz_engine_search_root": (C.c_int, [vp, C.c_uint64, C.c_uint64, C.c_int, C.c_int, C.c_int, i32p, f32p]),
    "rz_write_play_data": (C.c_int, [C.c_char_p, C.POINTER(Game), sz, C.POINTER(Ply), C.c_int, C.c_int, C.POINTER(sz)]),
    "rz_write_play_rows": (C.c_int, [C.c_char_p, C.POINTER(Game), sz, C.POINTER(Ply), C.c_int, C.c_int, C.POINTER(sz)]),
    "rz_read_play_rows": (C.c_int, [C.c_char_p, vp, sz, C.POINTER(sz), C.POINTER(C.c_int), C.POINTER(C.c_int)]),
    "rz_ingest_dev": (C.c_int, [vp, sz, C.c_int, C.c_int, vp, vp, vp, vp]),
    "rz_ingest": (C.c_int, [vp, sz, C.c_int, C.c_int, u8p, f32p, f32p]),
    "rz_ingest_json_dev": (C.c_int, [vp, sz, sz, vp, vp, vp, C.POINTER(sz), C.POINTER(sz), vp]),
    "rz_ingest_json_host": (C.c_int, [vp, sz, sz, vp, vp, vp, C.POINTER(sz), C.POINTER(sz)]),
    "rz_ingest_json": (C.c_int, [C.c_char_p, sz, vp, vp, vp, C.POINTER(sz), C.POINTER(sz)]),
    "rz_trainer_create": (C.c_int, [C.POINTER(NetCfg), C.POINTER(TrainCfg), C.c_int, C.POINTER(vp)]),
    "rz_trainer_create_group": (C.c_int, [C.POINTER(NetCfg), C.POINTER(TrainCfg), i32p, C.c_int, C.POINTER(vp)]),
    "rz_train_shard_plan_host": (C.c_int, [C.c_int, C.c_int, C.c_int, C.c_int, i32p]),
    "rz_trainer_destroy": (C.c_int, [vp]),
    "rz_trainer_blob_size": (C.c_int, [vp, C.POINTER(sz)]),
    "rz_trainer_load_weights": (C.c_int, [vp, f32p, sz]),
    "rz_trainer_load_weights_dev": (C.c_int, [vp, vp, sz, vp]),
    "rz_trainer_weights_dev": (C.c_int, [vp, vp, sz, vp]),
    "rz_trainer_step_dev": (C.c_int, [vp, vp, vp, vp, sz, vp, sz, C.c_float, vp, vp]),
    "rz_trainer_last_grad_dev": (C.c_int, [vp, vp, sz, vp]),
    "rz_trainer_replica_state_dev": (C.c_int, [vp, C.c_int, vp, vp, sz, vp]),
    "rz_trainer_debug_conv_dev": (C.c_int, [vp, C.c_int, vp, vp, vp, vp, sz, vp, vp]),
    "rz_trainer_debug_tensor_dev": (C.c_int, [vp, C.c_int, C.c_int, vp, sz, vp]),
    "rz_trainer_debug_keep_backward": (C.c_int, [vp, C.c_int]),
}

_lib = None


def lib():
    global _lib
    if _lib is None:
        if not os.path.exists(LIB_PATH):
            raise RzError(f"{LIB_PATH} not found: run `python -c 'import __graft_entry__ as g; g.build()'` "
                          f"(the CUDA extension is mandatory, there is no CPU fallback)")
        l = C.CDLL(LIB_PATH)
        for name, (res, args) in SIGNATURES.items():
            fn = getattr(l, name, None)
            if fn is not None:
                fn.restype, fn.argtypes = res, args
        _lib = l
    return _lib


def check(rc, what=""):
    if rc != 0:
        msg = lib().rz_last_error()
        raise RzError(f"{what} failed ({rc}): {msg.decode() if msg else ''}")
```

reversi-alpha-zero_b200/reversi_zero_b200/net.py:

```python
import ctypes as C

import numpy as np

from . import _cabi
from .agent import model as M

IMPL_AUTO, IMPL_GENERIC, IMPL_TCGEN05, IMPL_SPLIT = 0, 1, 2, 3


def set_tower_cluster(cluster):
    _cabi.check(_cabi.lib().rz_net_set_tower_cluster(int(cluster)), "rz_net_set_tower_cluster")


class Net:
    def __init__(self, model_config, device=0):
        self.mc = model_config
        self.device = device
        self._h = C.c_void_p()
        cfg = _cabi.NetCfg(model_config.cnn_filter_num, model_config.res_layer_num, model_config.value_fc_size,
                           model_config.cnn_filter_size)
        _cabi.check(_cabi.lib().rz_net_create(C.byref(cfg), device, C.byref(self._h)), "rz_net_create")
        n = C.c_size_t()
        _cabi.check(_cabi.lib().rz_net_blob_size(self._h, C.byref(n)), "rz_net_blob_size")
        self.blob_floats = n.value
        assert self.blob_floats == M.blob_size(model_config)
        self.digest = None

    @property
    def handle(self):
        return self._h

    def load_blob(self, blob):
        blob = np.ascontiguousarray(blob, dtype=np.float32)
        _cabi.check(_cabi.lib().rz_net_load_weights(self._h, blob.ctypes.data_as(_cabi.f32p), blob.size), "rz_net_load_weights")
        self.digest = M.blob_digest(blob)

    def load_weights(self, weights):
        self.load_blob(M.weights_to_blob(self.mc, weights))

    def load_blob_dev(self, tensor, stream_ptr=None):
        _cabi.check(_cabi.lib().rz_net_load_weights_dev(self._h, C.c_void_p(tensor.data_ptr()), tensor.numel(), stream_ptr),
                    "rz_net_load_weights_dev")

    def predict_planes(self, planes, impl=IMPL_AUTO):
        planes = np.ascontiguousarray(planes, dtype=np.uint8)
        n = planes.shape[0]
        policy = np.empty((n, 64), np.float32)
        value = np.empty((n,), np.float32)
        _cabi.check(_cabi.lib().rz_net_predict(self._h, planes.ctypes.data_as(_cabi.u8p), policy.ctypes.data_as(_cabi.f32p),
                                                value.ctypes.data_as(_cabi.f32p), n, impl), "rz_net_predict")
        return policy, value

    def predict_dev(self, own_t, enemy_t, policy_t, value_t, n, impl=IMPL_AUTO, stream_ptr=None):
        _cabi.check(_cabi.lib().rz_net_predict_dev(self._h, C.c_void_p(own_t.data_ptr()), C.c_void_p(enemy_t.data_ptr()),
                                                    C.c_void_p(policy_t.data_ptr()), C.c_void_p(value_t.data_ptr()), n, impl,
                                                    stream_ptr), "rz_net_predict_dev")

    def predict_counted_dev(self, own_t, enemy_t, policy_t, value_t, count_t, max_n, impl=IMPL_AUTO, stream_ptr=None):
        _cabi.check(_cabi.lib().rz_net_predict_counted_dev(self._h, C.c_void_p(own_t.data_ptr()), C.c_void_p(enemy_t.data_ptr()),
                                                            C.c_void_p(policy_t.data_ptr()), C.c_void_p(value_t.data_ptr()),
                                                            C.c_void_p(count_t.data_ptr()), max_n, impl, stream_ptr),
                    "rz_net_predict_counted_dev")

    def debug_tower_dev(self, own_t, enemy_t, policy_t, value_t, tower_t, n, stream_ptr=None):
        _cabi.check(_cabi.lib().rz_net_debug_tower_dev(self._h, C.c_void_p(own_t.data_ptr()), C.c_void_p(enemy_t.data_ptr()),
                                                        C.c_void_p(policy_t.data_ptr()), C.c_void_p(value_t.data_ptr()),
                                                        C.c_void_p(tower_t.data_ptr()), n, stream_ptr), "rz_net_debug_tower_dev")

    def debug_heads_dev(self, own_t, enemy_t, policy_t, value_t, logits_t, vlogit_t, n, tower_t=None, stream_ptr=None):
        _cabi.check(_cabi.lib().rz_net_debug_heads_dev(self._h, C.c_void_p(own_t.data_ptr()), C.c_void_p(enemy_t.data_ptr()),
                                                        C.c_void_p(policy_t.data_ptr()), C.c_void_p(value_t.data_ptr()),
                                                        C.c_void_p(tower_t.data_ptr()) if tower_t is not None else None,
                                                        C.c_void_p(logits_t.data_ptr()), C.c_void_p(vlogit_t.data_ptr()), n, stream_ptr),
                    "rz_net_debug_heads_dev")

    def debug_heads_impl_dev(self, own_t, enemy_t, policy_t, value_t, logits_t, vlogit_t, n, impl, tower_t=None, stream_ptr=None):
        _cabi.check(_cabi.lib().rz_net_debug_heads_impl_dev(
            self._h, C.c_void_p(own_t.data_ptr()), C.c_void_p(enemy_t.data_ptr()), C.c_void_p(policy_t.data_ptr()),
            C.c_void_p(value_t.data_ptr()), C.c_void_p(tower_t.data_ptr()) if tower_t is not None else None,
            C.c_void_p(logits_t.data_ptr()), C.c_void_p(vlogit_t.data_ptr()), n, int(impl), stream_ptr), "rz_net_debug_heads_impl_dev")

    def select_impl(self, n):
        impl = C.c_int()
        _cabi.check(_cabi.lib().rz_net_select_impl(self._h, n, C.byref(impl)), "rz_net_select_impl")
        return impl.value

    def close(self):
        if self._h:
            _cabi.lib().rz_net_destroy(self._h)
            self._h = C.c_void_p()

    def __del__(self):
        try:
            self.close()
        except Exception:
            pass
```

Before: 24.01.

## Add ping-pong warpgroup tower schedule and stage layer-0 weights through pipeline

Adds an optional ping-pong schedule for the wgmma residual tower, selected by a new setter or environment variable. Each math warpgroup processes its own board with its own named barrier, and the second warpgroup lags the first via a bar.arrive/bar.sync hand-off so the tensor-core work of the two groups interleaves. The activation layout is interleaved per board, and the pipeline deepens to four stages. The default lockstep path also changes: layer-0 weights now stream through the common stage ring instead of a dedicated buffer, the layer-0 operand is built directly in the activation buffer, and the first residual slots are kept in shared memory instead of global scratch. This adds complexity and per-warpgroup copies of scale/shift data, and it uses more shared memory.

New measurement: 24.28, median of 6. 1.1% higher.

```diff
diff --git a/include/rz_engine.h b/include/rz_engine.h
--- a/include/rz_engine.h
+++ b/include/rz_engine.h
@@ -80,6 +80,9 @@
 #define RZ_NET_IMPL_SPLIT 3
 
 int rz_net_set_tower_cluster(int cluster);
+#define RZ_TOWER_LOCKSTEP 0
+#define RZ_TOWER_PINGPONG 1
+int rz_net_set_tower_schedule(int schedule);
 int rz_net_create(const rz_net_cfg* cfg, int device, rz_net** out);
 int rz_net_destroy(rz_net* net);
 int rz_net_blob_size(const rz_net* net, size_t* n_floats);
diff --git a/reversi-alpha-zero_b200/csrc/rz_net.cu b/reversi-alpha-zero_b200/csrc/rz_net.cu
--- a/reversi-alpha-zero_b200/csrc/rz_net.cu
+++ b/reversi-alpha-zero_b200/csrc/rz_net.cu
@@ -303,6 +303,7 @@
 }
 
 int rz_net_set_tower_cluster(int cluster) { return set_tower_cluster(cluster); }
+int rz_net_set_tower_schedule(int schedule) { return set_tower_schedule(schedule); }
 
 int rz_net_predict_dev(rz_net* net, const uint64_t* own, const uint64_t* enemy, float* policy, float* value, size_t n, int impl,
                        void* stream) {
diff --git a/reversi-alpha-zero_b200/csrc/rz_net.cuh b/reversi-alpha-zero_b200/csrc/rz_net.cuh
--- a/reversi-alpha-zero_b200/csrc/rz_net.cuh
+++ b/reversi-alpha-zero_b200/csrc/rz_net.cuh
@@ -53,6 +53,8 @@
 inline bool tc_width(int filters) { return filters == 64 || filters == 128 || filters == 256; }
 int set_tower_cluster(int cluster);
 int tower_cluster();
+int set_tower_schedule(int schedule);
+int tower_schedule();
 int net_forward(rz_net* net, const uint64_t* own, const uint64_t* enemy, float* policy, float* value, size_t n, int impl,
                 cudaStream_t stream);
 
diff --git a/reversi-alpha-zero_b200/csrc/rz_net_tc.cu b/reversi-alpha-zero_b200/csrc/rz_net_tc.cu
--- a/reversi-alpha-zero_b200/csrc/rz_net_tc.cu
+++ b/reversi-alpha-zero_b200/csrc/rz_net_tc.cu
@@ -1,4 +1,5 @@
 #include <stdlib.h>
+#include <string.h>
 #include <mutex>
 #include <type_traits>
 #include "rz_bitboard.cuh"
@@ -11,23 +12,29 @@
 constexpr int kThreads = 384;
 constexpr uint32_t kProducerRegs = 40, kMathRegs = 232;
 constexpr int kMathThreads = 256;
-constexpr uint32_t kActCg = 2896, kActSlot = 144;
-constexpr uint32_t kActBytes = 32 * kActCg;
+constexpr uint32_t kActSlot = 144, kActCg = 18 * kActSlot;
+constexpr uint32_t kActBytes = 31 * kActCg + 20 * kActSlot + 16;
 constexpr uint32_t kStageBytes = 32768, kStages = 3;
 constexpr int kResAhead = 4;
-constexpr uint32_t kA0Bytes = 8192, kW0Bytes = 16384;
-constexpr uint32_t kOffAct = 0;
-constexpr uint32_t kOffW = kOffAct + kActBytes;
-constexpr uint32_t kOffA0 = kOffW + kStages * kStageBytes;
-constexpr uint32_t kOffW0 = kOffA0 + kA0Bytes;
-constexpr uint32_t kOffSS = kOffW0 + kW0Bytes;
+constexpr uint32_t kW0Bytes = 16384;
+constexpr uint32_t kOffW = (kActBytes + 127) & ~127u;
+constexpr int kResSmem = 10;
+constexpr uint32_t kOffSS = kOffW + kStages * kStageBytes;
 constexpr uint32_t kOffHw = kOffSS + 2 * 2048;
 constexpr uint32_t kOffBar = kOffHw + 768 * 4;
-constexpr uint32_t kNumBars = 2 * kStages + 1;
-constexpr uint32_t kSmemBytes = kOffBar + kNumBars * 8;
-constexpr uint32_t kSmemAlloc = kSmemBytes + 128;
+constexpr uint32_t kOffRes = (kOffBar + 2 * kStages * 8 + 127) & ~127u;
+constexpr uint32_t kSmemAlloc = kOffRes + kResSmem * kMathThreads * 16 + 128;
 static_assert(kSmemAlloc <= 232448, "shared memory budget exceeded");
 static_assert(kTowerResFloatsPerCta == (size_t)kMathThreads * 128, "residual scratch per CTA");
+
+constexpr uint32_t kPpStages = 4;
+constexpr uint32_t kPpOffSS = kOffW + kPpStages * kStageBytes;
+constexpr uint32_t kPpOffHw = kPpOffSS + 2 * 2 * 2048;
+constexpr uint32_t kPpOffBar = kPpOffHw + 768 * 4;
+constexpr uint32_t kPpSmemAlloc = kPpOffBar + 2 * kPpStages * 8 + 128;
+static_assert(kPpSmemAlloc <= 232448, "shared memory budget exceeded");
+constexpr int kLagStages = kPpStages - 2;
+static_assert(kLagStages > 0 && kLagStages < 4, "the hand-off is arrived at inside a layer's first tap");
 
 #ifdef RZ_TOWER_STAMPS
 enum : int {
@@ -43,8 +50,15 @@
     kStEpiLast,
     kStFeat,
     kStEmpty,
+    kStLag,
+    kStLagWait,
+    kStFull1,
+    kStEpiWg1,
+    kStHidden0,
+    kStHidden1,
     kStCount
 };
+constexpr int kStMaxLayers = 64;
 constexpr int kStMaxCtas = 1024;
 __device__ unsigned long long g_tower_stamps[kStMaxCtas][kStCount];
 __device__ __forceinline__ void stamp_add(int phase, uint32_t cycles) { atomicAdd(&g_tower_stamps[blockIdx.x][phase], (unsigned long long)cycles); }
@@ -53,31 +67,37 @@
 #define RZ_STAMP(...)
 #endif
 
-template <int CL>
+template <int CL, bool PP>
 __global__ void __launch_bounds__(kThreads, 1) net_tower_kernel(const Params pp) {
+    constexpr uint32_t kRowStep = PP ? 2 * kActSlot : kActSlot;
+    constexpr uint32_t kNStages = PP ? kPpStages : kStages;
+    constexpr uint32_t kSS = PP ? kPpOffSS : kOffSS, kHw = PP ? kPpOffHw : kOffHw;
+    constexpr int kResS = PP ? 0 : kResSmem;
+    constexpr uint32_t kBar = PP ? kPpOffBar : kOffBar;
     Params p = pp;
     if (p.n_dev) p.n = *p.n_dev;
     extern __shared__ uint8_t smem_raw[];
     const uint32_t base = (smem_u32(smem_raw) + 127u) & ~127u;
     uint8_t* sm = smem_raw + (base - smem_u32(smem_raw));
     const int warp = threadIdx.x >> 5, lane = threadIdx.x & 31;
-    const uint32_t bar0 = base + kOffBar;
+    const uint32_t bar0 = base + kBar;
     auto bar_full = [&](uint32_t s) { return bar0 + s * 8; };
-    auto bar_empty = [&](uint32_t s) { return bar0 + (kStages + s) * 8; };
-    const uint32_t bar_w0 = bar0 + 2 * kStages * 8;
+    auto bar_empty = [&](uint32_t s) { return bar0 + (kNStages + s) * 8; };
     const uint32_t ntiles = (p.n + 1) >> 1;
     const int L = p.n_layers;
     const uint32_t crank = CL > 1 ? cluster_ctarank() : 0u;
     const uint32_t cbase = blockIdx.x - crank;
     const uint32_t iters = cbase < ntiles ? (ntiles - cbase + gridDim.x - 1) / gridDim.x : 0u;
-
-    for (uint32_t i = threadIdx.x * 16; i < kActBytes; i += kThreads * 16) *reinterpret_cast<uint4*>(sm + kOffAct + i) = make_uint4(0, 0, 0, 0);
+#ifdef RZ_TOWER_STAMPS
+    __shared__ uint32_t st_lead[3][kStMaxLayers];
+#endif
+
+    for (uint32_t i = threadIdx.x * 16; i < kActBytes; i += kThreads * 16) *reinterpret_cast<uint4*>(sm + i) = make_uint4(0, 0, 0, 0);
     fence_proxy_async();
     for (uint32_t i = threadIdx.x; i < 768; i += kThreads)
-        reinterpret_cast<float*>(sm + kOffHw)[i] = __ldg(i < 512 ? p.blob + p.off_policy_conv + i : p.blob + p.off_value_conv + (i - 512));
+        reinterpret_cast<float*>(sm + kHw)[i] = __ldg(i < 512 ? p.blob + p.off_policy_conv + i : p.blob + p.off_value_conv + (i - 512));
     if (threadIdx.x == 0) {
-        for (uint32_t s = 0; s < kStages; ++s) { mbar_init(bar_full(s), 1); mbar_init(bar_empty(s), 8 * CL); }
-        mbar_init(bar_w0, 1);
+        for (uint32_t s = 0; s < kNStages; ++s) { mbar_init(bar_full(s), 1); mbar_init(bar_empty(s), 8 * CL); }
         asm volatile("fence.mbarrier_init.release.cluster;" ::: "memory");
     }
     __syncthreads();
@@ -86,28 +106,29 @@
     if (warp >= 8) {
         asm volatile("setmaxnreg.dec.sync.aligned.u32 %0;" ::"n"(kProducerRegs));
         if (warp == 8 && lane == 0) {
-            if (iters > 0) {
-                mbar_expect_tx(bar_w0, kW0Bytes);
-                bulk_g2s(base + kOffW0, p.w0, kW0Bytes, bar_w0);
-            }
             uint32_t stage = 0, phase = 0;
+            auto push = [&](const uint8_t* src, uint32_t bytes) {
+                mbar_wait(bar_empty(stage), phase ^ 1);
+                mbar_expect_tx(bar_full(stage), bytes);
+                if (CL == 1) {
+                    bulk_g2s(base + kOffW + stage * kStageBytes, src, bytes, bar_full(stage));
+                } else {
+                    const uint32_t slice = bytes / CL;
+                    bulk_g2s_mc(base + kOffW + stage * kStageBytes + crank * slice, src + crank * slice, slice, bar_full(stage),
+                                (uint16_t)((1u << CL) - 1u));
+                }
+                if (++stage == kNStages) { stage = 0; phase ^= 1; }
+            };
             for (uint32_t it = 0; it < iters; ++it) {
+                push(reinterpret_cast<const uint8_t*>(p.w0), kW0Bytes);
                 for (int l = 1; l < L; ++l) {
                     const uint8_t* src = reinterpret_cast<const uint8_t*>(p.w) + (size_t)(l - 1) * 36 * kStageBytes;
                     RZ_STAMP(uint32_t st_empty = 0;)
                     for (int s = 0; s < 36; ++s) {
                         RZ_STAMP(const uint32_t c0 = (uint32_t)clock();)
-                        mbar_wait(bar_empty(stage), phase ^ 1);
+                        RZ_STAMP(mbar_wait(bar_empty(stage), phase ^ 1);)
                         RZ_STAMP(st_empty += (uint32_t)clock() - c0;)
-                        mbar_expect_tx(bar_full(stage), kStageBytes);
-                        if (CL == 1) {
-                            bulk_g2s(base + kOffW + stage * kStageBytes, src + (size_t)s * kStageBytes, kStageBytes, bar_full(stage));
-                        } else {
-                            constexpr uint32_t kSlice = kStageBytes / CL;
-                            bulk_g2s_mc(base + kOffW + stage * kStageBytes + crank * kSlice, src + (size_t)s * kStageBytes + crank * kSlice,
-                                        kSlice, bar_full(stage), (uint16_t)((1u << CL) - 1u));
-                        }
-                        if (++stage == kStages) { stage = 0; phase ^= 1; }
+                        push(src + (size_t)s * kStageBytes, kStageBytes);
                     }
                     RZ_STAMP(stamp_add(kStEmpty, st_empty);)
                 }
@@ -117,60 +138,97 @@
         asm volatile("setmaxnreg.inc.sync.aligned.u32 %0;" ::"n"(kMathRegs));
         const int et = threadIdx.x;
         const int wg = warp >> 2;
-        const int r0 = wg * 64 + (warp & 3) * 16 + (lane >> 2);
-        const int g0 = r0 >> 3, x = r0 & 7, y = g0 >> 1;
         const int cq = 2 * (lane & 3);
-        const uint32_t act_row0 = base + kOffAct + (g0 + 2) * kActSlot + (x + 1) * 16 + cq * 2;
-        const uint32_t act_row1 = act_row0 + kActSlot;
-        const uint32_t a_wg = base + kOffAct + wg * 8 * kActSlot;
-        float* ss_s = reinterpret_cast<float*>(sm + kOffSS);
-        float4* res = reinterpret_cast<float4*>(p.res + (size_t)blockIdx.x * kTowerResFloatsPerCta) + et;
-        const float* hw = reinterpret_cast<const float*>(sm + kOffHw);
+        const int x = lane >> 2;
+        const int y = PP ? (warp & 3) * 2 : wg * 4 + (warp & 3);
+        const uint32_t act_row0 = PP ? base + (2 * (y + 1) + wg) * kActSlot + (x + 1) * 16 + cq * 2
+                                     : base + (2 * y + 2) * kActSlot + (x + 1) * 16 + cq * 2;
+        const uint32_t act_row1 = act_row0 + (PP ? 2 * kActSlot : kActSlot);
+        const uint32_t a_wg = base + (PP ? wg * kActSlot : wg * 8 * kActSlot);
+        float* ss_s = reinterpret_cast<float*>(sm + kSS) + (PP ? wg * 1024 : 0);
+        auto ss_copy = [&](uint32_t buf, size_t layer) {
+            const uint32_t dst = smem_u32(ss_s + buf * 512);
+            const float* src = p.ss + layer * 512;
+            if (PP) {
+                const int t = et & 127;
+#pragma unroll
+                for (int k = 0; k < 4; ++k) cp_async_4(dst + (t + 128 * k) * 4, src + t + 128 * k);
+            } else {
+                cp_async_4(dst + et * 4, src + et);
+                cp_async_4(dst + et * 4 + 1024, src + 256 + et);
+            }
+        };
+        float4* res_g = reinterpret_cast<float4*>(p.res + (size_t)blockIdx.x * kTowerResFloatsPerCta) + et;
+        float4* res_s = reinterpret_cast<float4*>(sm + kOffRes) + et;
+        auto res_at = [&](int i) { return i < kResS ? res_s + i * 256 : res_g + i * 256; };
+        const float* hw = reinterpret_cast<const float*>(sm + kHw);
         uint32_t stage = 0, phase = 0, ss_buf = 0;
         float d[128];
-        ss_s[et] = __ldg(p.ss + et);
-        ss_s[256 + et] = __ldg(p.ss + 256 + et);
+        ss_copy(0, 0);
+        cp_async_wait_all();
+        auto math_bar = [&]() {
+            if (PP) wg_bar(wg);
+            else epi_bar();
+        };
+        auto release = [&](uint32_t s) {
+            if (lane == 0) {
+                mbar_arrive(bar_empty(s));
+                if (CL > 1) mbar_arrive_cta(bar_empty(s), crank ^ 1u);
+            }
+        };
+        RZ_STAMP(const bool st_on = et == 0 || (PP && et == 128);)
+        RZ_STAMP(uint32_t st_k1_prev = 0, st_e0_prev = 0, st_e1_prev = 0;)
 
         for (uint32_t it = 0; it < iters; ++it) {
             const uint32_t tile = blockIdx.x + it * gridDim.x;
             const uint32_t pos0 = tile * 2;
             RZ_STAMP(const uint32_t st_tile0 = (uint32_t)clock();)
-            {
+            math_bar();
+            if (PP) {
+                const int t = et & 127, m = t & 63;
+                const bool valid = pos0 + wg < p.n;
+                build_layer0_row(sm + (2 * ((m >> 3) + 1) + wg) * kActSlot + ((m & 7) + 1) * 16, kActCg, valid ? p.own[pos0 + wg] : 0,
+                                 valid ? p.enemy[pos0 + wg] : 0, 2 * (t >> 6), m & 7, m >> 3);
+            } else {
                 const int m = et & 127, g = m >> 3, brd = g & 1;
                 const bool valid = pos0 + brd < p.n;
-                build_layer0_operand(sm + kOffA0, valid ? p.own[pos0 + brd] : 0, valid ? p.enemy[pos0 + brd] : 0, 2 * (et >> 7), g, m & 7,
-                                     g >> 1);
-                fence_proxy_async();
-            }
+                build_layer0_row(sm + (g + 2) * kActSlot + ((m & 7) + 1) * 16, kActCg, valid ? p.own[pos0 + brd] : 0,
+                                 valid ? p.enemy[pos0 + brd] : 0, 2 * (et >> 7), m & 7, g >> 1);
+            }
+            fence_proxy_async();
             float hs[6];
             for (int l = 0; l < L; ++l) {
                 const float* sc = ss_s + ss_buf * 512;
                 const bool is_conv2 = l > 0 && (l & 1) == 0;
                 float4 rb[kResAhead];
-                RZ_STAMP(uint32_t st_c = (uint32_t)clock(), st_bar = 0, st_full = 0, st_mma = 0;)
-                epi_bar();
+                RZ_STAMP(uint32_t st_c = (uint32_t)clock(), st_bar = 0, st_full = 0, st_mma = 0, st_lagw = 0;)
+                math_bar();
                 RZ_STAMP(st_bar += (uint32_t)clock() - st_c;)
-                {
-                    const size_t nl = l + 1 < L ? (size_t)l + 1 : 0;
-                    const uint32_t dst = smem_u32(ss_s + (ss_buf ^ 1) * 512 + et);
-                    cp_async_4(dst, p.ss + nl * 512 + et);
-                    cp_async_4(dst + 1024, p.ss + nl * 512 + 256 + et);
-                }
+                if (PP && wg == 1 && l > 0) {
+                    RZ_STAMP(st_c = (uint32_t)clock();)
+                    lag_wait();
+                    RZ_STAMP(st_lagw = (uint32_t)clock() - st_c;)
+                }
+                ss_copy(ss_buf ^ 1, l + 1 < L ? (size_t)l + 1 : 0);
                 RZ_STAMP(const uint32_t st_k0 = (uint32_t)clock();)
+                RZ_STAMP(if (PP && et == 0) reinterpret_cast<volatile uint32_t*>(&st_lead[0][0])[l & (kStMaxLayers - 1)] = st_k0;)
                 acc_fence(d);
                 if (l == 0) {
                     RZ_STAMP(st_c = (uint32_t)clock();)
-                    mbar_wait(bar_w0, 0);
+                    mbar_wait(bar_full(stage), phase);
+                    const uint32_t a0 = a_wg + 2 * kActSlot + 16, b0 = base + kOffW + stage * kStageBytes;
                     RZ_STAMP(st_full += (uint32_t)clock() - st_c;)
                     wgmma_fence();
 #pragma unroll
                     for (uint32_t j = 0; j < 2; ++j)
-                        wgmma_m64n256k16(d, smem_desc(base + kOffA0 + j * 2 * 2048 + wg * 1024, 2048, 128),
-                                         smem_desc(base + kOffW0 + j * 2 * 4096, 4096, 128), j);
+                        wgmma_m64n256k16(d, smem_desc(a0 + j * 2 * kActCg, kActCg, kRowStep),
+                                         smem_desc(b0 + j * 2 * 4096, 4096, 128), j);
                     wgmma_commit();
                     RZ_STAMP(st_c = (uint32_t)clock();)
                     wgmma_wait<0>();
                     RZ_STAMP(st_mma += (uint32_t)clock() - st_c;)
+                    release(stage);
+                    if (++stage == kNStages) { stage = 0; phase ^= 1; }
                 } else {
                     int prev = -1;
                     for (uint32_t tap = 0; tap < 9; ++tap) {
@@ -183,31 +241,26 @@
                             wgmma_fence();
 #pragma unroll
                             for (uint32_t j = 0; j < 4; ++j)
-                                wgmma_m64n256k16(d, smem_desc(a_tap + (kb * 8 + 2 * j) * kActCg, kActCg, kActSlot),
+                                wgmma_m64n256k16(d, smem_desc(a_tap + (kb * 8 + 2 * j) * kActCg, kActCg, kRowStep),
                                                  smem_desc(b_st + 2 * j * 4096, 4096, 128), (tap | kb | j) != 0);
                             wgmma_commit();
+                            if (PP && wg == 0 && tap == 0 && kb == kLagStages) lag_arrive();
                             RZ_STAMP(st_c = (uint32_t)clock();)
                             wgmma_wait<1>();
                             RZ_STAMP(st_mma += (uint32_t)clock() - st_c;)
-                            if (prev >= 0 && lane == 0) {
-                                mbar_arrive(bar_empty(prev));
-                                if (CL > 1) mbar_arrive_cta(bar_empty(prev), crank ^ 1u);
-                            }
+                            if (prev >= 0) release((uint32_t)prev);
                             prev = (int)stage;
-                            if (++stage == kStages) { stage = 0; phase ^= 1; }
+                            if (++stage == kNStages) { stage = 0; phase ^= 1; }
                         }
                     }
                     if (is_conv2) {
 #pragma unroll
-                        for (int i = 0; i < kResAhead; ++i) rb[i] = res[i * 256];
+                        for (int i = 0; i < kResAhead; ++i) rb[i] = *res_at(i);
                     }
                     RZ_STAMP(st_c = (uint32_t)clock();)
                     wgmma_wait<0>();
                     RZ_STAMP(st_mma += (uint32_t)clock() - st_c;)
-                    if (lane == 0) {
-                        mbar_arrive(bar_empty(prev));
-                        if (CL > 1) mbar_arrive_cta(bar_empty(prev), crank ^ 1u);
-                    }
+                    release((uint32_t)prev);
                 }
                 RZ_STAMP(const uint32_t st_k1 = (uint32_t)clock();)
                 acc_fence(d);
@@ -216,13 +269,20 @@
                 const bool keep_res = l == 0 || is_conv2;
                 const bool last = l == L - 1;
                 RZ_STAMP(st_c = (uint32_t)clock();)
-                if (!last) epi_bar();
+                if (!last) math_bar();
                 RZ_STAMP(const uint32_t st_e0 = (uint32_t)clock(); st_bar += st_e0 - st_c;)
                 float* dbg0 = nullptr;
                 float* dbg1 = nullptr;
                 if (last && p.dbg_tower) {
-                    if (pos0 < p.n) dbg0 = p.dbg_tower + ((size_t)pos0 * 64 + y * 8 + x) * 256;
-                    if (pos0 + 1 < p.n) dbg1 = p.dbg_tower + ((size_t)(pos0 + 1) * 64 + y * 8 + x) * 256;
+                    if (PP) {
+                        if (pos0 + wg < p.n) {
+                            dbg0 = p.dbg_tower + ((size_t)(pos0 + wg) * 64 + y * 8 + x) * 256;
+                            dbg1 = dbg0 + 8 * 256;
+                        }
+                    } else {
+                        if (pos0 < p.n) dbg0 = p.dbg_tower + ((size_t)pos0 * 64 + y * 8 + x) * 256;
+                        if (pos0 + 1 < p.n) dbg1 = p.dbg_tower + ((size_t)(pos0 + 1) * 64 + y * 8 + x) * 256;
+                    }
                 }
                 constexpr int kEpiRelu = 0, kEpiKeep = 1, kEpiLast = 2;
                 auto epilogue = [&](auto conv2, auto kind) {
@@ -241,14 +301,14 @@
                     float v2 = fmaf(d[4 * i + 2], s.x, b.x), v3 = fmaf(d[4 * i + 3], s.y, b.y);
                     if (kConv2) {
                         const float4 r = rb[i % kResAhead];
-                        if (i + kResAhead < 32) rb[i % kResAhead] = res[(i + kResAhead) * 256];
+                        if (i + kResAhead < 32) rb[i % kResAhead] = *res_at(i + kResAhead);
                         v0 += r.x; v1 += r.y; v2 += r.z; v3 += r.w;
                     }
                     if (kKeep || kLast) {
                         v0 = fmaxf(v0, 0.f); v1 = fmaxf(v1, 0.f); v2 = fmaxf(v2, 0.f); v3 = fmaxf(v3, 0.f);
                     }
                     if (!kLast) {
-                        if (kKeep) res[i * 256] = make_float4(v0, v1, v2, v3);
+                        if (kKeep) *res_at(i) = make_float4(v0, v1, v2, v3);
                         const uint32_t h0 = pack_h2<!kKeep>(v0, v1);
                         const uint32_t h1 = pack_h2<!kKeep>(v2, v3);
                         const uint32_t off = (c >> 3) * kActCg;
@@ -281,9 +341,33 @@
                     epilogue(NoConv2(), std::integral_constant<int, kEpiRelu>());
                 }
                 if (!last) fence_proxy_async();
-                RZ_STAMP(if (et == 0) {
-                    stamp_add(kStKLoop, st_k1 - st_k0); stamp_add(kStFull, st_full); stamp_add(kStMma, st_mma); stamp_add(kStEpiBar, st_bar);
-                    stamp_add(l == 0 ? kStEpi0 : last ? kStEpiLast : is_conv2 ? kStEpi2 : kStEpi1, (uint32_t)clock() - st_e0);
+                RZ_STAMP(if (st_on) {
+                    const uint32_t st_e1 = (uint32_t)clock();
+                    if (et == 0) {
+                        stamp_add(kStKLoop, st_k1 - st_k0); stamp_add(kStFull, st_full); stamp_add(kStMma, st_mma); stamp_add(kStEpiBar, st_bar);
+                        stamp_add(l == 0 ? kStEpi0 : last ? kStEpiLast : is_conv2 ? kStEpi2 : kStEpi1, st_e1 - st_e0);
+                        if (PP) {
+                            volatile uint32_t* lead = &st_lead[0][0];
+                            lead[kStMaxLayers + (l & (kStMaxLayers - 1))] = st_e0;
+                            lead[2 * kStMaxLayers + (l & (kStMaxLayers - 1))] = st_e1;
+                        }
+                    } else {
+                        stamp_add(kStFull1, st_full);
+                        stamp_add(kStLagWait, st_lagw);
+                        if (!last) stamp_add(kStEpiWg1, st_e1 - st_e0);
+                        if (l > 0) {
+                            const volatile uint32_t* lead = &st_lead[0][0];
+                            const uint32_t lk0 = lead[l & (kStMaxLayers - 1)];
+                            const uint32_t le0 = lead[kStMaxLayers + ((l - 1) & (kStMaxLayers - 1))];
+                            const uint32_t le1 = lead[2 * kStMaxLayers + ((l - 1) & (kStMaxLayers - 1))];
+                            stamp_add(kStLag, st_k0 - lk0);
+                            const int h0 = min((int)(st_k1_prev - le0), (int)(le1 - le0));
+                            const int h1 = (int)(st_e1_prev - st_e0_prev) - max((int)(lk0 - st_e0_prev), 0);
+                            stamp_add(kStHidden0, h0 > 0 ? (uint32_t)h0 : 0u);
+                            stamp_add(kStHidden1, h1 > 0 ? (uint32_t)h1 : 0u);
+                        }
+                        st_k1_prev = st_k1; st_e0_prev = st_e0; st_e1_prev = st_e1;
+                    }
                 })
             }
             RZ_STAMP(const uint32_t st_h0 = (uint32_t)clock();)
@@ -294,10 +378,11 @@
             }
             {
                 const int q = lane & 3;
-                if (q < 2 && pos0 + q < p.n) {
+                const uint32_t pos = PP ? pos0 + wg : pos0 + q;
+                if (q < 2 && pos < p.n) {
                     const float h0 = q ? hs[3] : hs[0], h1 = q ? hs[4] : hs[1], h2 = q ? hs[5] : hs[2];
-                    store_head_features(p.feat + (size_t)(pos0 + q) * kHeadFeatures, p.ss + (size_t)L * 512, y * 8 + x, h0 + 0.f,
-                                        h1 + 0.f, h2 + 0.f);
+                    store_head_features(p.feat + (size_t)pos * kHeadFeatures, p.ss + (size_t)L * 512, (PP ? y + q : y) * 8 + x,
+                                        h0 + 0.f, h1 + 0.f, h2 + 0.f);
                 }
             }
             RZ_STAMP(if (et == 0) {
@@ -354,6 +439,40 @@
     return g_cluster;
 }
 
+static int g_schedule = -1;
+
+int set_tower_schedule(int schedule) {
+    RZ_REQUIRE(schedule == RZ_TOWER_LOCKSTEP || schedule == RZ_TOWER_PINGPONG, "rz_net_set_tower_schedule: unknown schedule %d", schedule);
+    g_schedule = schedule;
+    return RZ_OK;
+}
+
+int tower_schedule() {
+    if (g_schedule < 0) {
+        const char* s = getenv("RZ_TOWER_SCHEDULE");
+        g_schedule = (s && strcmp(s, "pingpong") == 0) ? RZ_TOWER_PINGPONG : RZ_TOWER_LOCKSTEP;
+    }
+    return g_schedule;
+}
+
+template <int CL, bool PP>
+static int launch_tower(const tc::Params& p, uint32_t grid, cudaStream_t stream) {
+    const uint32_t smem = PP ? tc::kPpSmemAlloc : tc::kSmemAlloc;
+    if (CL == 1) {
+        tc::net_tower_kernel<1, PP><<<grid, tc::kThreads, smem, stream>>>(p);
+    } else {
+        cudaLaunchConfig_t cfg = {};
+        cfg.gridDim = dim3(grid); cfg.blockDim = dim3(tc::kThreads); cfg.dynamicSmemBytes = smem; cfg.stream = stream;
+        cudaLaunchAttribute attr[1];
+        attr[0].id = cudaLaunchAttributeClusterDimension;
+        attr[0].val.clusterDim.x = 2; attr[0].val.clusterDim.y = 1; attr[0].val.clusterDim.z = 1;
+        cfg.attrs = attr; cfg.numAttrs = 1;
+        RZ_CUDA_TRY(cudaLaunchKernelEx(&cfg, tc::net_tower_kernel<2, PP>, p));
+    }
+    RZ_LAUNCH_CHECK();
+    return RZ_OK;
+}
+
 int net_forward_tc(rz_net* net, const uint64_t* own, const uint64_t* enemy, float* policy, float* value, size_t n, cudaStream_t stream,
                    float* dbg_tower, const uint32_t* n_dev, float* dbg_logits, float* dbg_vlogit) {
     if (net->cfg.filters == 64 || net->cfg.filters == 128)
@@ -361,19 +480,26 @@
     RZ_REQUIRE(net->cfg.filters == 256, "wgmma tower requires 64, 128 or 256 filters (got %d)", net->cfg.filters);
     RZ_REQUIRE(net->cfg.value_fc <= (int)tc::kTcMaxV, "wgmma tower supports value_fc_size <= %u", tc::kTcMaxV);
     RZ_REQUIRE(n < (1ull << 31), "batch too large");
-    static int max_pairs = -1;
-    if (max_pairs < 0) {
-        RZ_CUDA_TRY(cudaFuncSetAttribute(tc::net_tower_kernel<1>, cudaFuncAttributeMaxDynamicSharedMemorySize, (int)tc::kSmemAlloc));
-        RZ_CUDA_TRY(cudaFuncSetAttribute(tc::net_tower_kernel<2>, cudaFuncAttributeMaxDynamicSharedMemorySize, (int)tc::kSmemAlloc));
+    static int max_pairs[2] = {-1, -1};
+    if (max_pairs[0] < 0) {
+        RZ_CUDA_TRY(cudaFuncSetAttribute(tc::net_tower_kernel<1, false>, cudaFuncAttributeMaxDynamicSharedMemorySize, (int)tc::kSmemAlloc));
+        RZ_CUDA_TRY(cudaFuncSetAttribute(tc::net_tower_kernel<2, false>, cudaFuncAttributeMaxDynamicSharedMemorySize, (int)tc::kSmemAlloc));
+        RZ_CUDA_TRY(cudaFuncSetAttribute(tc::net_tower_kernel<1, true>, cudaFuncAttributeMaxDynamicSharedMemorySize, (int)tc::kPpSmemAlloc));
+        RZ_CUDA_TRY(cudaFuncSetAttribute(tc::net_tower_kernel<2, true>, cudaFuncAttributeMaxDynamicSharedMemorySize, (int)tc::kPpSmemAlloc));
         cudaLaunchConfig_t cfg = {};
-        cfg.gridDim = dim3((unsigned)num_sms() & ~1u); cfg.blockDim = dim3(tc::kThreads); cfg.dynamicSmemBytes = tc::kSmemAlloc;
+        cfg.gridDim = dim3((unsigned)num_sms() & ~1u); cfg.blockDim = dim3(tc::kThreads);
         cudaLaunchAttribute attr[1];
         attr[0].id = cudaLaunchAttributeClusterDimension;
         attr[0].val.clusterDim.x = 2; attr[0].val.clusterDim.y = 1; attr[0].val.clusterDim.z = 1;
         cfg.attrs = attr; cfg.numAttrs = 1;
-        RZ_CUDA_TRY(cudaOccupancyMaxActiveClusters(&max_pairs, tc::net_tower_kernel<2>, &cfg));
-    }
-    const int cluster = tower_cluster() == 2 && max_pairs >= 1 ? 2 : 1;
+        cfg.dynamicSmemBytes = tc::kSmemAlloc;
+        RZ_CUDA_TRY(cudaOccupancyMaxActiveClusters(&max_pairs[0], tc::net_tower_kernel<2, false>, &cfg));
+        cfg.dynamicSmemBytes = tc::kPpSmemAlloc;
+        RZ_CUDA_TRY(cudaOccupancyMaxActiveClusters(&max_pairs[1], tc::net_tower_kernel<2, true>, &cfg));
+    }
+    const bool pp = tower_schedule() == RZ_TOWER_PINGPONG;
+    const int pairs = max_pairs[pp];
+    const int cluster = tower_cluster() == 2 && pairs >= 1 ? 2 : 1;
     tc::Params p;
     p.w0 = net->tc_w0; p.w = net->tc_w; p.ss = net->scale_shift; p.blob = net->blob;
     p.off_policy_conv = net->off_policy_conv; p.off_policy_fc_k = net->off_policy_fc_k; p.off_policy_fc_b = net->off_policy_fc_b;
@@ -389,20 +515,12 @@
     RZ_CUDA_TRY(cudaStreamWaitEvent(stream, net->res_done, 0));
     const uint32_t ntiles = (uint32_t)((n + 1) / 2);
     uint32_t grid = ntiles < (uint32_t)num_sms() ? ntiles : (uint32_t)num_sms();
-    if (cluster == 1) {
-        tc::net_tower_kernel<1><<<grid, tc::kThreads, tc::kSmemAlloc, stream>>>(p);
-    } else {
+    if (cluster == 2) {
         grid = (grid + 1) & ~1u;
-        if (grid > 2u * (uint32_t)max_pairs) grid = 2u * (uint32_t)max_pairs;
-        cudaLaunchConfig_t cfg = {};
-        cfg.gridDim = dim3(grid); cfg.blockDim = dim3(tc::kThreads); cfg.dynamicSmemBytes = tc::kSmemAlloc; cfg.stream = stream;
-        cudaLaunchAttribute attr[1];
-        attr[0].id = cudaLaunchAttributeClusterDimension;
-        attr[0].val.clusterDim.x = 2; attr[0].val.clusterDim.y = 1; attr[0].val.clusterDim.z = 1;
-        cfg.attrs = attr; cfg.numAttrs = 1;
-        RZ_CUDA_TRY(cudaLaunchKernelEx(&cfg, tc::net_tower_kernel<2>, p));
-    }
-    RZ_LAUNCH_CHECK();
+        if (grid > 2u * (uint32_t)pairs) grid = 2u * (uint32_t)pairs;
+    }
+    auto launch = cluster == 1 ? (pp ? launch_tower<1, true> : launch_tower<1, false>) : (pp ? launch_tower<2, true> : launch_tower<2, false>);
+    RZ_TRY(launch(p, grid, stream));
     RZ_TRY(net_heads(p, stream));
     RZ_CUDA_TRY(cudaEventRecord(net->res_done, stream));
     return RZ_OK;
diff --git a/reversi-alpha-zero_b200/csrc/rz_tc_common.cuh b/reversi-alpha-zero_b200/csrc/rz_tc_common.cuh
--- a/reversi-alpha-zero_b200/csrc/rz_tc_common.cuh
+++ b/reversi-alpha-zero_b200/csrc/rz_tc_common.cuh
@@ -65,6 +65,9 @@
 __device__ __forceinline__ void cp_async_wait_all() { asm volatile("cp.async.wait_all;" ::: "memory"); }
 __device__ __forceinline__ void fence_proxy_async() { asm volatile("fence.proxy.async.shared::cta;" ::: "memory"); }
 __device__ __forceinline__ void epi_bar() { asm volatile("bar.sync 1, 256;" ::: "memory"); }
+__device__ __forceinline__ void wg_bar(int wg) { asm volatile("bar.sync %0, 128;" ::"r"(2 + wg) : "memory"); }
+__device__ __forceinline__ void lag_arrive() { asm volatile("bar.arrive 4, 256;" ::: "memory"); }
+__device__ __forceinline__ void lag_wait() { asm volatile("bar.sync 4, 256;" ::: "memory"); }
 
 __device__ __forceinline__ uint64_t smem_desc(uint32_t addr, uint32_t lbo, uint32_t sbo) {
     return (uint64_t)((addr >> 4) & 0x3FFF) | ((uint64_t)((lbo >> 4) & 0x3FFF) << 16) | ((uint64_t)((sbo >> 4) & 0x3FFF) << 32);
@@ -161,7 +164,7 @@
 
 constexpr uint32_t kTcMaxV = 512;
 
-__device__ __forceinline__ void build_layer0_operand(uint8_t* a0, u64 o, u64 e, int kc0, int g, int x, int y) {
+__device__ __forceinline__ void build_layer0_row(uint8_t* row, uint32_t kc_stride, u64 o, u64 e, int kc0, int x, int y) {
 #pragma unroll
     for (int kk = 0; kk < 2; ++kk) {
         const int kc = kc0 + kk;
@@ -181,8 +184,11 @@
             }
             w[jp] = packed;
         }
-        *reinterpret_cast<uint4*>(a0 + kc * 2048 + g * 128 + x * 16) = make_uint4(w[0], w[1], w[2], w[3]);
+        *reinterpret_cast<uint4*>(row + kc * kc_stride) = make_uint4(w[0], w[1], w[2], w[3]);
     }
+}
+__device__ __forceinline__ void build_layer0_operand(uint8_t* a0, u64 o, u64 e, int kc0, int g, int x, int y) {
+    build_layer0_row(a0 + g * 128 + x * 16, 2048, o, e, kc0, x, y);
 }
 
 __device__ __forceinline__ void store_head_features(float* f, const float* ssh, int pix, float a0, float a1, float av) {
diff --git a/reversi-alpha-zero_b200/reversi_zero_b200/_cabi.py b/reversi-alpha-zero_b200/reversi_zero_b200/_cabi.py
--- a/reversi-alpha-zero_b200/reversi_zero_b200/_cabi.py
+++ b/reversi-alpha-zero_b200/reversi_zero_b200/_cabi.py
@@ -95,6 +95,7 @@
     "rz_net_predict_dev": (C.c_int, [vp, vp, vp, vp, vp, sz, C.c_int, vp]),
     "rz_net_predict_counted_dev": (C.c_int, [vp, vp, vp, vp, vp, vp, sz, C.c_int, vp]),
     "rz_net_set_tower_cluster": (C.c_int, [C.c_int]),
+    "rz_net_set_tower_schedule": (C.c_int, [C.c_int]),
     "rz_net_debug_tower_dev": (C.c_int, [vp, vp, vp, vp, vp, vp, sz, vp]),
     "rz_net_debug_heads_dev": (C.c_int, [vp, vp, vp, vp, vp, vp, vp, vp, sz, vp]),
     "rz_net_debug_heads_impl_dev": (C.c_int, [vp, vp, vp, vp, vp, vp, vp, vp, sz, C.c_int, vp]),
diff --git a/reversi-alpha-zero_b200/reversi_zero_b200/net.py b/reversi-alpha-zero_b200/reversi_zero_b200/net.py
--- a/reversi-alpha-zero_b200/reversi_zero_b200/net.py
+++ b/reversi-alpha-zero_b200/reversi_zero_b200/net.py
@@ -10,6 +10,13 @@
 
 def set_tower_cluster(cluster):
     _cabi.check(_cabi.lib().rz_net_set_tower_cluster(int(cluster)), "rz_net_set_tower_cluster")
+
+
+TOWER_LOCKSTEP, TOWER_PINGPONG = 0, 1
+
+
+def set_tower_schedule(schedule):
+    _cabi.check(_cabi.lib().rz_net_set_tower_schedule(int(schedule)), "rz_net_set_tower_schedule")
 
 
 class Net:
```
